# illuin-tech/colpali

Measured on AMD Instinct MI355X. Metric: MaxSim (query,doc) pairs scored/sec, higher is better.
Workload: dtype bf16; 1 GPU; 4 query x 32 tokens vs resident pre-embedded shard of 125000 docs x 1024 patches x d=128 bf16 per GPU (30.5 GiB/GPU), fused MaxSim + per-shard top-10; docs_per_gpu=125000, doc_len=1024, n_queries=4, q_len=32, top_k=10, parallelism=corpus-sharded x1

## Files before the change

colpali_amd/_lib.py:

```python
from __future__ import annotations

import ctypes
import os

import torch

_HERE = os.path.dirname(os.path.abspath(__file__))
_AB_DIR = os.path.realpath(os.path.join(_HERE, "..", "tools", "_ab"))


def _lib_path() -> str:
    override = os.environ.get("COLPALI_AMD_LIB")
    if override:
        real = os.path.realpath(override)
        if os.path.dirname(real) != _AB_DIR:
            raise RuntimeError(f"COLPALI_AMD_LIB={override}: only measurement builds under {_AB_DIR} can replace the in-tree library")
        return real
    return os.path.join(_HERE, "csrc", "libmaxsim_gfx950.so")


LIB_PATH = _lib_path()

MSIM_FLAG_REF_ROUNDING = 0x1
ABI_VERSION = 22


def dtype_code(dtype) -> int:
    if dtype == torch.bfloat16:
        return 0
    if dtype == torch.float16:
        return 1
    if dtype == torch.float32:
        return 2
    raise NotImplementedError(f"dtype {dtype}: the gfx950 kernels take bfloat16, float16 or float32 embeddings")


def kernel_width(dim: int, dtype) -> int:
    es = 4 if dtype == torch.float32 else 2
    if es == 2 and dim == 128:
        return dim
    per = 32 // es
    width = (dim + per - 1) // per * per
    if width * es > 4096:
        raise NotImplementedError(f"embedding rows of {dim} x {es} bytes exceed the 4 KiB the gfx950 kernels support")
    return width

_lib = None


class MaxSimLibraryError(RuntimeError):
    pass


def lib() -> ctypes.CDLL:
    global _lib
    if _lib is not None:
        return _lib
    if not os.path.exists(LIB_PATH):
        raise MaxSimLibraryError(
            f"{LIB_PATH} is missing: build it with `python -c 'import __graft_entry__ as g; g.build()'` "
            "(or `make -C colpali_amd/csrc`). colpali_amd has no CPU/torch fallback."
        )
    L = ctypes.CDLL(LIB_PATH)
    vp, i32, i64, u32, sz = ctypes.c_void_p, ctypes.c_int, ctypes.c_int64, ctypes.c_uint32, ctypes.c_size_t
    L.msim_abi_version.restype = i32
    L.msim_last_error.restype = ctypes.c_char_p
    L.msim_fwd_workspace_bytes.argtypes = [i32, i32, i32, i32, i32]
    L.msim_fwd_workspace_bytes.restype = sz
    L.msim_fwd.argtypes = [i32, vp, i32, i32, vp, vp, vp, i32, i32, vp, i64, u32, vp, vp]
    L.msim_fwd.restype = i32
    L.msim_fwd_host.argtypes = [i32, vp, i32, i32, vp, vp, vp, i32, i32, vp, i64, u32, i32]
    L.msim_fwd_host.restype = i32
    L.msim_host_last_error.restype = ctypes.c_char_p
    L.msim_fwd_host_lists.argtypes = [i32, vp, vp, i32, vp, vp, vp, i32, i32, vp, i64, u32, i32]
    L.msim_fwd_host_lists.restype = i32
    L.msim_sim_matrix_host.argtypes = [i32, vp, i32, vp, i32, i32, vp, i64, u32, i32]
    L.msim_sim_matrix_host.restype = i32
    L.msim_fwd_plan.argtypes = [vp, i32, i32, vp]
    L.msim_fwd_plan.restype = i32
    L.msim_fwd_ragged_workspace_bytes.argtypes = [i32, vp, i32, i32, i32]
    L.msim_fwd_ragged_workspace_bytes.restype = sz
    L.msim_fwd_ragged.argtypes = [i32, vp, vp, vp, i32, vp, vp, vp, i32, i32, vp, i64, u32, vp, vp]
    L.msim_fwd_ragged.restype = i32
    L.msim_query_compact.argtypes = [vp, i32, i32, i32, vp, vp, vp, vp]
    L.msim_query_compact.restype = i32
    L.msim_host_count_nonzero_rows.argtypes = [vp, vp, i64, i64, vp, i32]
    L.msim_host_count_nonzero_rows.restype = i32
    L.msim_host_gather_nonzero_rows.argtypes = [vp, vp, vp, i64, vp, i64, i32]
    L.msim_host_gather_nonzero_rows.restype = i32
    L.msim_fwd_transposed.argtypes = [i32, vp, i32, i32, vp, i32, i32, i32, vp, i64, vp, vp]
    L.msim_fwd_transposed.restype = i32
    L.msim_dense_t_supported.argtypes = [i32, i32, i32, i32, i32, i32]
    L.msim_dense_t_supported.restype = i32
    L.msim_dense_t_route_bytes.argtypes = [i32, i32, i32]
    L.msim_dense_t_route_bytes.restype = sz
    L.msim_fwd_transposed_route.argtypes = [i32, vp, i32, i32, vp, i32, i32, i32, vp, i64, vp, vp, vp]
    L.msim_fwd_transposed_route.restype = i32
    L.msim_dense_t_bwd_workspace_bytes.argtypes = [i32, i32, i32, i32, i32]
    L.msim_dense_t_bwd_workspace_bytes.restype = sz
    L.msim_dense_t_bwd.argtypes = [i32, vp, i32, i32, vp, i32, i32, i32, vp, i64, vp, i32, vp, vp, vp, vp, vp]
    L.msim_dense_t_bwd.restype = i32
    L.msim_host_gather_range.argtypes = [vp, vp, vp, i64, i64, i64, i32]
    L.msim_host_gather_range.restype = i32
    L.msim_host_gather_range_begin.argtypes = [vp, vp, vp, i64, i64, i64, i32]
    L.msim_host_gather_range_begin.restype = i32
    L.msim_host_gather_range_wait.argtypes = []
    L.msim_host_gather_range_wait.restype = i32
    L.msim_host_threads_affinity.argtypes = [vp, i32]
    L.msim_host_threads_affinity.restype = i32
    L.msim_pairs_argmax.argtypes = [i32, vp, i32, i32, vp, vp, vp, i32, i32, i32, vp, i32, vp, vp, vp]
    L.msim_pairs_argmax.restype = i32
    L.msim_allpairs_argmax.argtypes = [i32, vp, i32, i32, vp, vp, vp, i32, i32, vp, i64, vp, vp]
    L.msim_allpairs_argmax.restype = i32
    L.msim_pairs_bwd.argtypes = [i32, vp, i32, i32, vp, vp, i32, i32, i32, vp, vp, vp, vp, i32, vp, i32, i32, vp, vp, vp, vp]
    L.msim_pairs_bwd.restype = i32
    L.msim_pairs_bwd_workspace_bytes.argtypes = [i32, i32, i32, i32, i32, i32]
    L.msim_pairs_bwd_workspace_bytes.restype = sz
    f32 = ctypes.c_float
    L.msim_smooth_fwd.argtypes = [i32, vp, i32, i32, vp, vp, i32, i32, f32, vp, i64, vp]
    L.msim_smooth_fwd.restype = i32
    L.msim_smooth_pairs.argtypes = [i32, vp, i32, i32, vp, vp, i32, i32, vp, i32, f32, vp, vp, vp]
    L.msim_smooth_pairs.restype = i32
    L.msim_smooth_bwd_workspace_bytes.argtypes = [i32, i32, i32]
    L.msim_smooth_bwd_workspace_bytes.restype = sz
    L.msim_smooth_pairs_bwd.argtypes = [i32, vp, i32, i32, vp, vp, i32, i32, i32, vp, vp, vp, vp, i32, f32, vp, vp, vp, vp]
    L.msim_smooth_pairs_bwd.restype = i32
    L.msim_embed_head.argtypes = [i32, vp, i64, i32, vp, vp, i32, vp, vp, i64, vp]
    L.msim_embed_head.restype = i32
    L.msim_embed_head_row_map.argtypes = [vp, i32, vp, i32, i64, vp, vp]
    L.msim_embed_head_row_map.restype = i32
    L.msim_embed_head_writer_map.argtypes = [vp, i32, vp, i32, i32, i32, vp, vp, vp, vp, vp]
    L.msim_embed_head_writer_map.restype = i32
    L.msim_embed_head_bwd.argtypes = [i32, vp, vp, vp, i64, i32, vp, vp]
    L.msim_embed_head_bwd.restype = i32
    L.msim_sim_matrix.argtypes = [i32, vp, i32, vp, i32, i32, vp, i64, u32, vp]
    L.msim_sim_matrix.restype = i32
    L.msim_pool_cluster.argtypes = [i32, vp, vp, i32, i32, i32, vp, i32, vp, vp, vp, vp, vp]
    L.msim_pool_cluster.restype = i32
    L.msim_pool_reduce.argtypes = [i32, vp, vp, i32, i32, i32, vp, vp, vp, i32, vp]
    L.msim_pool_reduce.restype = i32
    L.msim_loss_epilogue_workspace_bytes.argtypes = [i32, i32]
    L.msim_loss_epilogue_workspace_bytes.restype = sz
    L.msim_loss_epilogue.argtypes = [i32, vp, i64, i32, i32, vp, i32, i32, i32, i32, f32, i32, i32, f32, f32, vp, vp, vp, vp, vp, vp, vp, vp, vp]
    L.msim_loss_epilogue.restype = i32
    L.msim_host_gather.argtypes = [vp, vp, vp, vp, i64, i32]
    L.msim_host_gather.restype = i32
    L.msim_fwd_candidates_workspace_bytes.argtypes = [i32, i32, i32]
    L.msim_fwd_candidates_workspace_bytes.restype = sz
    L.msim_fwd_candidates.argtypes = [i32, vp, vp, vp, i32, vp, vp, vp, i32, i32, vp, i32, i64, i64, vp, i64, vp, u32, vp, vp]
    L.msim_fwd_candidates.restype = i32
    L.msim_fwd_candidates_wide_workspace_bytes.argtypes = [i32, i32, i32, i32]
    L.msim_fwd_candidates_wide_workspace_bytes.restype = sz
    L.msim_fwd_candidates_wide.argtypes = L.msim_fwd_candidates.argtypes
    L.msim_fwd_candidates_wide.restype = i32
    L.msim_fde_encode_docs.argtypes = [i32, vp, vp, i32, i64, i32, vp, vp, i32, i32, i32, i32, vp, vp, vp]
    L.msim_fde_encode_docs.restype = i32
    L.msim_fde_encode_queries.argtypes = [i32, vp, vp, i32, i64, i32, vp, vp, i32, i32, i32, vp, vp, vp]
    L.msim_fde_encode_queries.restype = i32
    L.msim_fde_scores.argtypes = [i32, vp, i32, vp, i32, i32, vp, i64, vp]
    L.msim_fde_scores.restype = i32
    L.msim_i8_encode_docs.argtypes = [i32, vp, vp, i32, i64, i32, vp, vp, vp]
    L.msim_i8_encode_docs.restype = i32
    L.msim_i8_encode_queries.argtypes = [i32, vp, i64, i32, vp, vp, vp]
    L.msim_i8_encode_queries.restype = i32
    L.msim_i8_scores.argtypes = [vp, vp, vp, i32, i64, i32, vp, vp, vp, vp, i32, i64, i32, vp, i64, vp]
    L.msim_i8_scores.restype = i32
    L.msim_cent_encode_docs.argtypes = [i32, vp, vp, i32, i64, i32, i32, vp, i32, vp, vp, vp]
    L.msim_cent_encode_docs.restype = i32
    L.msim_cent_table_bytes.argtypes = [i32, i32, i32]
    L.msim_cent_table_bytes.restype = sz
    L.msim_cent_table.argtypes = [i32, vp, vp, i32, i64, i32, i32, vp, i32, vp, vp]
    L.msim_cent_table.restype = i32
    L.msim_cent_scores_plan.argtypes = [i32, i32, i32, i32, i64, vp]
    L.msim_cent_scores_plan.restype = i32
    L.msim_cent_scores.argtypes = [vp, vp, i32, i64, i32, i32, vp, vp, vp, i32, i64, vp, i64, vp]
    L.msim_cent_scores.restype = i32
    L.msim_res_encode_docs.argtypes = [i32, vp, i64, i32, vp, vp, i32, vp, i32, vp, vp]
    L.msim_res_encode_docs.restype = i32
    L.msim_res_decode_rows.argtypes = [i32, vp, vp, i64, i64, i64, vp, i32, vp, i32, i32, vp, vp]
    L.msim_res_decode_rows.restype = i32
    L.msim_res_candidates_workspace_bytes.argtypes = [i32, i32, i32]
    L.msim_res_candidates_workspace_bytes.restype = sz
    L.msim_res_candidates.argtypes = [i32, vp, vp, vp, i32, vp, vp, vp, i32, vp, i32, vp, vp, i32, i64, i32, vp, i32, i64, i64, vp, i64,
                                      vp, vp, vp]
    L.msim_res_candidates.restype = i32
    L.msim_res_scores_workspace_bytes.argtypes = [i32, i32]
    L.msim_res_scores_workspace_bytes.restype = sz
    L.msim_res_scores.argtypes = [i32, vp, vp, vp, i32, vp, vp, vp, i32, vp, i32, vp, vp, i32, i64, i32, vp, i64, vp, vp]
    L.msim_res_scores.restype = i32
    L.msim_live_compact_workspace_bytes.argtypes = [i32, i64]
    L.msim_live_compact_workspace_bytes.restype = sz
    L.msim_live_compact.argtypes = [vp, i64, i64, vp, vp, i32, vp, vp, vp, i64, vp]
    L.msim_live_compact.restype = i32
    L.msim_live_mask_scores.argtypes = [vp, i64, i32, i64, vp, vp]
    L.msim_live_mask_scores.restype = i32
    L.msim_mine_bounds.argtypes = [vp, i64, i32, i64, vp, vp, i64, i64, vp, i32, vp, vp]
    L.msim_mine_bounds.restype = i32
    L.msim_mine_mask.argtypes = [vp, i64, i32, i64, vp, f32, vp, vp, vp, i64, i64, vp]
    L.msim_mine_mask.restype = i32
    L.msim_gather_pages.argtypes = [vp, i64, i64, vp, i32, i64, vp, i64, i64, vp, vp, vp]
    L.msim_gather_pages.restype = i32
    L.msim_filter_pack.argtypes = [vp, i64, i32, i64, vp, i64, vp]
    L.msim_filter_pack.restype = i32
    L.msim_filter_mask.argtypes = [vp, i64, i32, i64, vp, i64, vp, vp, vp, vp]
    L.msim_filter_mask.restype = i32
    L.msim_filter_list_workspace_bytes.argtypes = [i32, i64]
    L.msim_filter_list_workspace_bytes.restype = sz
    L.msim_filter_list.argtypes = [vp, i64, vp, vp, vp, i32, i64, i64, vp, i64, i32, vp, vp, vp]
    L.msim_filter_list.restype = i32
    L.msim_filter_ids.argtypes = [vp, i64, i32, i64, i64, i64, vp, i64, vp, vp, vp, vp]
    L.msim_filter_ids.restype = i32
    L.msim_group_reduce.argtypes = [vp, i64, i32, i64, vp, vp, i32, i64, vp, vp, i64, vp]
    L.msim_group_reduce.restype = i32
    L.msim_group_select.argtypes = [vp, vp, vp, i32, i32, i64, i32, vp, vp, vp, vp]
    L.msim_group_select.restype = i32
    L.msim_align_candidates.argtypes =[i32, vp, vp, i32, i64, i32, vp, vp, vp, i32, i64, i32, vp, i32, i64, i64, vp, vp, vp, i32, vp]
    L.msim_align_candidates.restype = i32
    L.msim_topk_workspace_bytes.argtypes = [i32, i64, i32]
    L.msim_topk_workspace_bytes.restype = sz
    L.msim_topk_f32.argtypes = [vp, vp, i32, i64, i64, i32, i64, vp, vp, vp, vp]
    L.msim_topk_f32.restype = i32
    if L.msim_abi_version() != ABI_VERSION:
        raise MaxSimLibraryError(f"ABI version mismatch: library reports {L.msim_abi_version()}, binding expects {ABI_VERSION} "
                                 "(rebuild: make -C colpali_amd/csrc)")
    _lib = L
    return L


def check(rc: int, what: str) -> None:
    if rc != 0:
        msg = lib().msim_last_error().decode("utf-8", "replace")
        if rc == -2:
            raise NotImplementedError(f"{what}: {msg}")
        if rc == -1:
            raise ValueError(f"{what}: {msg}")
        raise MaxSimLibraryError(f"{what} failed (code {rc}): {msg}")


class StreamConstCache:

    def __init__(self, capacity: int):
        import collections
        import threading

        self._d = collections.OrderedDict()
        self._lock = threading.Lock()
        self._cap = capacity

    def get(self, key, device, make):
        k = (key, str(device), torch.cuda.current_stream(device).cuda_stream if torch.device(device).type == "cuda" else 0)
        with self._lock:
            t = self._d.get(k)
            if t is not None:
                self._d.move_to_end(k)
                return t
        t = make()
        with self._lock:
            self._d[k] = t
            while len(self._d) > self._cap:
                self._d.popitem(last=False)
        return t

    def __len__(self):
        return len(self._d)


def effective_cpus() -> int:
    try:
        n = len(os.sched_getaffinity(0))
    except Exception:
        n = os.cpu_count() or 1
    quota = None
    try:
        q, p = open("/sys/fs/cgroup/cpu.max").read().split()[:2]
        if q != "max":
            quota = int(q) / int(p)
    except Exception:
        try:
            q = int(open("/sys/fs/cgroup/cpu/cpu.cfs_quota_us").read())
            p = int(open("/sys/fs/cgroup/cpu/cpu.cfs_period_us").read())
            if q > 0 and p > 0:
                quota = q / p
        except Exception:
            pass
    if quota is not None:
        n = min(n, max(1, int(quota)))
    return max(1, n)


_gpu_cpus = {}


def _parse_cpulist(text: str):
    cpus = set()
    for part in text.strip().split(","):
        if not part:
            continue
        lo, _, hi = part.partition("-")
        cpus.update(range(int(lo), int(hi or lo) + 1))
    return cpus


def gpu_local_cpus(device):
    idx = device.index if getattr(device, "index", None) is not None else torch.cuda.current_device()
    if idx in _gpu_cpus:
        return _gpu_cpus[idx]
    cpus = None
    if os.environ.get("COLPALI_AMD_NUMA", "1") != "0":
        try:
            p = torch.cuda.get_device_properties(idx)
            bus = f"{p.pci_domain_id:04x}:{p.pci_bus_id:02x}:{p.pci_device_id:02x}.0"
            local = _parse_cpulist(open(f"/sys/bus/pci/devices/{bus}/local_cpulist").read())
            allowed = os.sched_getaffinity(0)
            local &= allowed
            if len(local) >= 2 and local != allowed:
                cpus = frozenset(local)
        except Exception:
            cpus = None
    _gpu_cpus[idx] = cpus
    return cpus


class on_gpu_local_cpus:

    def __init__(self, device):
        self.cpus = gpu_local_cpus(device) if torch.cuda.is_available() else None
        self.saved = None

    def __enter__(self):
        if self.cpus is not None:
            try:
                saved = os.sched_getaffinity(0)
                if saved != self.cpus:
                    os.sched_setaffinity(0, self.cpus)
                    self.saved = saved
            except Exception:
                self.saved = None
        return self

    def __exit__(self, *exc):
        if self.saved is not None:
            try:
                os.sched_setaffinity(0, self.saved)
            except Exception:
                pass
        return False


_SYS_MOVE_PAGES = 279


def nodes_of_addresses(addrs) -> list:
    try:
        n = len(addrs)
        if n == 0:
            return []
        libc = ctypes.CDLL(None, use_errno=True)
        pages = (ctypes.c_void_p * n)(*[int(a) & ~4095 for a in addrs])
        status = (ctypes.c_int * n)()
        libc.syscall.restype = ctypes.c_long
        rc = libc.syscall(ctypes.c_long(_SYS_MOVE_PAGES), ctypes.c_int(0), ctypes.c_ulong(n), pages, ctypes.c_void_p(0), status, ctypes.c_int(0))
        if rc != 0:
            return []
        return [int(x) for x in status if x >= 0]
    except Exception:
        return []


_node_cpus = {}


def node_cpus(node: int):
    if node in _node_cpus:
        return _node_cpus[node]
    cpus = None
    try:
        local = _parse_cpulist(open(f"/sys/devices/system/node/node{node}/cpulist").read()) & os.sched_getaffinity(0)
        if len(local) >= 2:
            cpus = frozenset(local)
    except Exception:
        cpus = None
    _node_cpus[node] = cpus
    return cpus


_gather_threads_on = [None]
GATHER_NODE_POLICY = os.environ.get("COLPALI_AMD_GATHER_NODE", "gpu")


def place_gather_threads(device, sample_addrs) -> None:
    if os.environ.get("COLPALI_AMD_NUMA", "1") == "0":
        return
    try:
        want = gpu_local_cpus(device)
        if GATHER_NODE_POLICY == "pages":
            nodes = nodes_of_addresses(sample_addrs)
            if nodes:
                node = max(set(nodes), key=nodes.count)
                want = node_cpus(node) or want
        if want is None or want == _gather_threads_on[0]:
            return
        arr = (ctypes.c_int32 * len(want))(*sorted(want))
        if lib().msim_host_threads_affinity(arr, len(want)) == 0:
            _gather_threads_on[0] = want
    except Exception:
        pass


def ptr(t) -> int:
    return 0 if t is None else t.data_ptr()


def current_stream_handle(device) -> int:
    return torch.cuda.current_stream(device).cuda_stream


def workspace(nbytes: int, device):
    return torch.empty((nbytes,), dtype=torch.uint8, device=device) if nbytes else None
```

colpali_amd/corpus.py:

```python
from __future__ import annotations

import ctypes
import operator
import os
import threading
from dataclasses import dataclass
from typing import List, Optional, Sequence, Union

import numpy as np
import torch

from . import _lib as _lib_mod
from ._lib import kernel_width

EMBED_DIM = 128


def block_clamp0(lengths: torch.Tensor, batch_size: int) -> torch.Tensor:
    if batch_size <= 0:
        raise ValueError("batch_size must be positive")
    import numpy as np

    ln = lengths.detach().to("cpu").numpy().astype(np.int64, copy=False)
    n = ln.size
    if n == 0:
        return torch.zeros((0,), dtype=torch.uint8)
    if batch_size >= n:
        flags = ln < ln.max()
    else:
        pad = (-n) % batch_size
        padded = np.concatenate([ln, np.full((pad,), -1, dtype=np.int64)]) if pad else ln
        block_max = np.repeat(padded.reshape(-1, batch_size).max(axis=1), batch_size)[:n]
        flags = ln < block_max
    return torch.from_numpy(flags.astype(np.uint8))


@dataclass
class PackedCorpus:
    blob: torch.Tensor
    offsets: torch.Tensor
    clamp0: Optional[torch.Tensor]
    lengths: torch.Tensor
    id_base: int = 0
    avg_rows: Optional[int] = None

    def __len__(self) -> int:
        return int(self.lengths.numel())

    def average_rows(self) -> int:
        if self.avg_rows is None:
            n = len(self)
            if not n:
                self.avg_rows = 0
            elif self.lengths.device.type == "cpu":
                self.avg_rows = int(self.lengths.numpy().sum(dtype=np.int64)) // n
            else:
                self.avg_rows = int(self.lengths.sum()) // n
        return self.avg_rows

    @property
    def device(self) -> torch.device:
        return self.blob.device

    @property
    def dtype(self) -> torch.dtype:
        return self.blob.dtype

    @property
    def width(self) -> int:
        return int(self.blob.shape[1])

    @property
    def nbytes(self) -> int:
        return self.blob.numel() * self.blob.element_size()


def _check_embeddings(x: torch.Tensor, what: str) -> None:
    if x.dim() not in (2, 3):
        raise ValueError(f"{what}: expected 2-D or 3-D embeddings")
    if x.dtype not in (torch.bfloat16, torch.float16, torch.float32):
        raise NotImplementedError(
            f"{what}: dtype {x.dtype}; the gfx950 kernels take bfloat16 (what the ColPali/ColQwen2 forward emits), "
            "float16 or float32 embeddings. Converting silently would change the scores, so this is an error.")
    kernel_width(x.shape[-1], x.dtype)


def _widen(x: torch.Tensor) -> torch.Tensor:
    width = kernel_width(x.shape[-1], x.dtype)
    if width == x.shape[-1]:
        return x
    return torch.nn.functional.pad(x, (0, width - x.shape[-1]))


def _env_int(name: str, default: int, lo: int, hi: int) -> int:
    try:
        return max(lo, min(hi, int(os.environ[name])))
    except (KeyError, ValueError):
        return default


_COPY_THREADS = _env_int("COLPALI_AMD_COPY_THREADS", max(1, min(8, _lib_mod.effective_cpus() // 2)), 1, 256)
_EDGE_CHUNK_BYTES = _env_int("COLPALI_AMD_EDGE_CHUNK_MB", 16, 0, 1024) << 20
_EDGE_LAST_BYTES = (lambda mb: -1 if mb < 0 else mb << 20)(_env_int("COLPALI_AMD_EDGE_LAST_MB", -1, -1, 1024))
STAGING_BYTES = _env_int("COLPALI_AMD_STAGING_MB", 64, 2, 16384) << 20
_ASYNC_GATHER = _env_int("COLPALI_AMD_ASYNC_GATHER", 1, 0, 1) == 1


class _Staging:

    def __init__(self):
        self.buf: Optional[torch.Tensor] = None
        self.events = [None, None]
        self.lock = threading.Lock()
        self.next_half = 0

    def _halves(self, want: int):
        half = max(min(want, STAGING_BYTES // 2), 1 << 20)
        if self.buf is None or self.buf.numel() < 2 * half:
            for ev in self.events:
                if ev is not None:
                    ev.synchronize()
            with _lib_mod.on_gpu_local_cpus(torch.device("cuda", torch.cuda.current_device()) if torch.cuda.is_available() else None):
                self.buf = torch.empty((2 * half,), dtype=torch.uint8, pin_memory=True)
        return self.buf.numel() // 2

    def upload(self, ps: Sequence[torch.Tensor], dim: int, device: torch.device,
               slot_rows: Optional[int] = None) -> torch.Tensor:
        dtype = ps[0].dtype
        es = ps[0].element_size()
        total = sum(int(p.shape[0]) for p in ps) if slot_rows is None else len(ps) * slot_rows
        nbytes = total * dim * es
        dev = torch.empty((total, dim), dtype=dtype, device=device)
        if nbytes == 0:
            return dev
        dev_bytes = dev.view(torch.uint8).view(-1)
        with self.lock:
            half = self._halves(nbytes)
            base = self.buf.data_ptr()
            import numpy as np

            L = _lib_mod.lib()
            keep, offs, srcs, sizes = [], [], [], []
            o = 0
            for p in ps:
                n = int(p.shape[0]) * dim * es
                if n:
                    src = p if p.is_contiguous() else p.contiguous()
                    keep.append(src)
                    sp, done = src.data_ptr(), 0
                    while done < n:
                        room = half - ((o + done) % half)
                        take = min(room, n - done)
                        offs.append(o + done)
                        srcs.append(sp + done)
                        sizes.append(take)
                        done += take
                o += n if slot_rows is None else slot_rows * dim * es
            offs_a = np.asarray(offs, dtype=np.int64)
            srcs_a = np.asarray(srcs, dtype=np.uint64)
            sizes_a = np.asarray(sizes, dtype=np.int64)
            stream = torch.cuda.current_stream(device)
            k = 0
            n_pieces = len(offs)
            for c0 in range(0, nbytes, half):
                c1 = min(nbytes, c0 + half)
                h = (c0 // half) & 1
                hb = base + h * half
                if self.events[h] is not None:
                    self.events[h].synchronize()
                if slot_rows is not None:
                    ctypes.memset(hb, 0, c1 - c0)
                k1 = k
                while k1 < n_pieces and offs[k1] < c1:
                    k1 += 1
                if k1 > k:
                    rel = offs_a[k:k1] - c0
                    rc = L.msim_host_gather(hb, srcs_a[k:k1].ctypes.data, rel.ctypes.data, sizes_a[k:k1].ctypes.data,
                                            k1 - k, _COPY_THREADS)
                    if rc != 0:
                        raise RuntimeError(f"msim_host_gather failed: {L.msim_last_error().decode()}")
                k = k1
                dev_bytes[c0:c1].copy_(self.buf[h * half : h * half + (c1 - c0)], non_blocking=True)
                self.events[h] = torch.cuda.Event()
                self.events[h].record(stream)
            del keep
        return dev


    def upload_image(self, srcs, prefix, n: int, dst_bytes: Optional[torch.Tensor], side_stream, on_chunk=None, prepare=None) -> None:
        total = int(prefix[n])
        if total == 0:
            if prepare is not None:
                prepare()
            return
        L = _lib_mod.lib()
        with self.lock:
            half = self._halves(total)
            base = self.buf.data_ptr()
            chunks = _chunk_schedule(total, half)
            in_flight = False

            def begin(k: int) -> int:
                h = self.next_half
                self.next_half ^= 1
                if self.events[h] is not None:
                    self.events[h].synchronize()
                c0, c1 = chunks[k]
                rc = L.msim_host_gather_range_begin(base + h * half, srcs.ctypes.data, prefix.ctypes.data, n, c0, c1, _COPY_THREADS)
                if rc != 0:
                    raise RuntimeError(f"msim_host_gather_range_begin failed: {L.msim_host_last_error().decode()}")
                return h

            try:
                if not _ASYNC_GATHER and prepare is not None:
                    got = prepare()
                    dst_bytes = got if dst_bytes is None else dst_bytes
                h = begin(0)
                in_flight = True
                if _ASYNC_GATHER and prepare is not None:
                    got = prepare()
                    dst_bytes = got if dst_bytes is None else dst_bytes
                for k, (c0, c1) in enumerate(chunks):
                    rc = L.msim_host_gather_range_wait()
                    in_flight = False
                    if rc != 0:
                        raise RuntimeError(f"msim_host_gather_range failed: {L.msim_host_last_error().decode()}")
                    with torch.cuda.stream(side_stream):
                        dst_bytes[c0:c1].copy_(self.buf[h * half : h * half + (c1 - c0)], non_blocking=True)
                        ev = torch.cuda.Event()
                        ev.record(side_stream)
                    self.events[h] = ev
                    if _ASYNC_GATHER and k + 1 < len(chunks):
                        h = begin(k + 1)
                        in_flight = True
                    if on_chunk is not None:
                        on_chunk(c1)
                    if not _ASYNC_GATHER and k + 1 < len(chunks):
                        h = begin(k + 1)
                        in_flight = True
            finally:
                if in_flight:
                    L.msim_host_gather_range_wait()


def _chunk_schedule(total: int, half: int):
    edge = min(_EDGE_CHUNK_BYTES, half)
    last = min(_EDGE_LAST_BYTES, half) if _EDGE_LAST_BYTES >= 0 else edge
    if edge <= 0 or last <= 0 or total <= 2 * half:
        return [(c0, min(total, c0 + half)) for c0 in range(0, total, half)]
    cuts = [0, edge]
    while total - cuts[-1] > half + last:
        cuts.append(cuts[-1] + half)
    if total - cuts[-1] > last:
        cuts.append(total - last)
    cuts.append(total)
    return list(zip(cuts[:-1], cuts[1:]))


class _PerDevice:

    def __init__(self):
        self._by_dev = {}
        self._lock = threading.Lock()

    def of(self, device) -> _Staging:
        idx = torch.device(device).index
        if idx is None:
            idx = torch.cuda.current_device() if torch.cuda.is_available() else -1
        with self._lock:
            st = self._by_dev.get(idx)
            if st is None:
                st = self._by_dev[idx] = _Staging()
            return st

    def upload(self, ps, dim, device, slot_rows=None):
        return self.of(device).upload(ps, dim, device, slot_rows)


_staging = _PerDevice()
_staging_q = _PerDevice()
_copy_streams = {}


def copy_stream(device: torch.device) -> torch.cuda.Stream:
    device = torch.device(device)
    key = device.index if device.index is not None else torch.cuda.current_device()
    st = _copy_streams.get(key)
    if st is None:
        st = _copy_streams[key] = torch.cuda.Stream(device=device)
    return st


_dim_of = torch.Tensor.dim
_dtype_of = operator.attrgetter("dtype")
_shape_of = operator.attrgetter("shape")
_is_cpu = operator.attrgetter("is_cpu")
_is_contig = torch.Tensor.is_contiguous
_data_ptr = torch.Tensor.data_ptr
_stride_of = torch.Tensor.stride
_numel_of = torch.Tensor.numel


def host_list_image(ps: Sequence[torch.Tensor], what: str = "passages"):
    first = ps[0]
    dtype, dim = first.dtype, (first.shape[1] if first.dim() == 2 else -1)
    if dim > 0 and type(ps) in (list, tuple):
        n = len(ps)
        if (set(map(_dim_of, ps)) == {2} and set(map(_dtype_of, ps)) == {dtype} and all(map(_is_cpu, ps))
                and all(map(_is_contig, ps)) and set(map(_stride_of, ps)) == {(dim, 1)}):
            numel = np.fromiter(map(_numel_of, ps), dtype=np.int64, count=n)
            rows = numel // dim
            if bool((rows >= 2).all()) and bool((rows * dim == numel).all()):
                _check_embeddings(first, what)
                srcs = np.fromiter(map(_data_ptr, ps), dtype=np.uint64, count=n)
                return list(ps), srcs, rows, int(dim), dtype
    keep = []
    for p in ps:
        if p.dim() != 2:
            raise ValueError(f"each {what[:-1]} must be 2-D (sequence_length, dim)")
        if p.dtype != dtype:
            raise RuntimeError(f"expected {what} of one dtype, got {dtype} and {p.dtype}")
        if p.shape[1] != dim:
            raise RuntimeError(f"expected {what} of one embedding width, got {dim} and {p.shape[1]}")
        if p.device.type != "cpu":
            return None
        keep.append(p if p.is_contiguous() else p.contiguous())
    _check_embeddings(first, what)
    srcs = np.fromiter((t.data_ptr() for t in keep), dtype=np.uint64, count=len(keep))
    rows = np.fromiter((t.shape[0] for t in keep), dtype=np.int64, count=len(keep))
    return keep, srcs, rows, int(dim), dtype


def _gather_rows(ps: Sequence[torch.Tensor], dim: int, device: torch.device) -> torch.Tensor:
    device = torch.device(device)
    if device.type == "cuda" and all(p.device.type == "cpu" for p in ps):
        return _staging.upload(ps, dim, device)
    return torch.cat([p.reshape(-1, dim) for p in ps], dim=0).to(device, non_blocking=True)


def pack_passages(ps: Union[torch.Tensor, Sequence[torch.Tensor]], device: torch.device,
                  batch_size: Optional[int] = 128, id_base: int = 0) -> PackedCorpus:
    if isinstance(ps, torch.Tensor):
        if ps.dim() != 3:
            raise ValueError("a passage tensor must be 3-D (n_passages, max_len, dim)")
        _check_embeddings(ps, "passages")
        n, L, dim = ps.shape
        blob = _widen(ps.reshape(n * L, dim).to(device, non_blocking=True)).contiguous()
        lengths = torch.full((n,), L, dtype=torch.int64)
        clamp0 = None
    else:
        if len(ps) == 0:
            raise ValueError("No passages provided")
        for p in ps:
            if p.dim() != 2:
                raise ValueError("each passage must be 2-D (sequence_length, dim)")
            _check_embeddings(p, "passages")
            if p.dtype != ps[0].dtype:
                raise RuntimeError(f"expected passages of one dtype, got {ps[0].dtype} and {p.dtype}")
            if p.shape[1] != ps[0].shape[1]:
                raise RuntimeError(f"expected passages of one embedding width, got {ps[0].shape[1]} and {p.shape[1]}")
        dim = ps[0].shape[1]
        lengths = torch.tensor([p.shape[0] for p in ps], dtype=torch.int64)
        blob = _widen(_gather_rows(ps, dim, device)).contiguous()
        clamp0 = None
        if batch_size is not None:
            flags = block_clamp0(lengths, batch_size)
            if bool(flags.any()):
                clamp0 = flags.to(device)
            if bool((lengths == 0).any()):
                for j in range(0, len(ps), batch_size):
                    if int(lengths[j : j + batch_size].max()) == 0:
                        raise RuntimeError("max(): Expected reduction dim 3 to have non-zero size.")
    if blob.numel() == 0:
        blob = torch.zeros((1, blob.shape[1]), dtype=blob.dtype, device=device)
    offsets = torch.zeros(lengths.numel() + 1, dtype=torch.int64)
    torch.cumsum(lengths, 0, out=offsets[1:])
    if int(offsets[-1]) >= 2**31:
        raise NotImplementedError("more than 2^31 patch rows in one shard")
    return PackedCorpus(blob=blob, offsets=offsets.to(torch.int32).to(device), clamp0=clamp0,
                        lengths=lengths, id_base=id_base)


@dataclass
class PackedQueries:
    tokens: torch.Tensor
    offsets: torch.Tensor
    offsets_host: torch.Tensor

    def __len__(self) -> int:
        return int(self.offsets_host.numel()) - 1

    @property
    def device(self) -> torch.device:
        return self.tokens.device

    @property
    def dtype(self) -> torch.dtype:
        return self.tokens.dtype

    @property
    def lengths(self) -> torch.Tensor:
        return (self.offsets_host[1:] - self.offsets_host[:-1]).to(torch.int64)

    def select(self, lo: int, hi: int) -> "PackedQueries":
        base = int(self.offsets_host[lo])
        oh = (self.offsets_host[lo:hi + 1] - base).contiguous()
        return PackedQueries(tokens=self.tokens[base:int(self.offsets_host[hi])] if hi > lo else self.tokens[:0],
                             offsets=oh.to(self.tokens.device, non_blocking=True), offsets_host=oh)


MAX_FLAT_QUERY_TOKENS = 1024
WIDE_DIM = 320
MAX_FLAT_QUERY_TOKENS_WIDE = 512


def _is_flat_shape(dtype: torch.dtype, dim: int) -> bool:
    return dtype in (torch.bfloat16, torch.float16) and dim in (EMBED_DIM, WIDE_DIM)


def max_flat_query_tokens(dim: int) -> int:
    return MAX_FLAT_QUERY_TOKENS_WIDE if dim == WIDE_DIM else MAX_FLAT_QUERY_TOKENS


def _flat_from_host_list(qs: Sequence[torch.Tensor], dim: int, device: torch.device, compact: bool) -> Optional["PackedQueries"]:
    import numpy as np

    L = _lib_mod.lib()
    es = qs[0].element_size()
    row_bytes = dim * es
    keep = [q if q.is_contiguous() else q.contiguous() for q in qs]
    n = len(keep)
    srcs = np.asarray([q.data_ptr() for q in keep], dtype=np.uint64)
    rows = np.asarray([int(q.shape[0]) for q in keep], dtype=np.int64)
    if compact:
        counts = np.zeros(n, dtype=np.int32)
        rc = L.msim_host_count_nonzero_rows(srcs.ctypes.data, rows.ctypes.data, row_bytes, n, counts.ctypes.data, _COPY_THREADS)
        if rc != 0:
            raise RuntimeError(f"msim_host_count_nonzero_rows failed: {L.msim_last_error().decode()}")
    else:
        counts = rows.astype(np.int32)
    if int(counts.max(initial=0)) > max_flat_query_tokens(dim):
        return None
    off = np.zeros(n + 1, dtype=np.int64)
    np.cumsum(counts, out=off[1:])
    total = int(off[-1])
    offsets_host = torch.from_numpy(off.astype(np.int32))
    tokens = torch.empty((max(total, 1), dim), dtype=qs[0].dtype, device=device)
    if total == 0:
        tokens.zero_()
    else:
        st = _staging_q.of(device)
        stream = torch.cuda.current_stream(device)
        dst_bytes = tokens.view(torch.uint8).view(-1)
        if not compact:
            prefix = np.zeros(n + 1, dtype=np.int64)
            np.cumsum(rows * row_bytes, out=prefix[1:])
            st.upload_image(srcs, prefix, n, dst_bytes[:total * row_bytes], stream)
        else:
            with st.lock:
                half = st._halves(total * row_bytes)
                base = st.buf.data_ptr()
                g0 = 0
                while g0 < n:
                    g1 = g0 + 1
                    while g1 < n and (off[g1 + 1] - off[g0]) * row_bytes <= half:
                        g1 += 1
                    nb = int(off[g1] - off[g0]) * row_bytes
                    if nb:
                        h = st.next_half
                        st.next_half ^= 1
                        if st.events[h] is not None:
                            st.events[h].synchronize()
                        dst_row = np.ascontiguousarray(off[g0:g1] - off[g0])
                        rc = L.msim_host_gather_nonzero_rows(base + h * half, srcs[g0:g1].ctypes.data, rows[g0:g1].ctypes.data, row_bytes,
                                                             dst_row.ctypes.data, g1 - g0, _COPY_THREADS)
                        if rc != 0:
                            raise RuntimeError(f"host query gather failed: {L.msim_last_error().decode()}")
                        lo = int(off[g0]) * row_bytes
                        dst_bytes[lo:lo + nb].copy_(st.buf[h * half: h * half + nb], non_blocking=True)
                        ev = torch.cuda.Event()
                        ev.record(stream)
                        st.events[h] = ev
                    g0 = g1
    del keep
    return PackedQueries(tokens=tokens, offsets=offsets_host.to(device, non_blocking=True), offsets_host=offsets_host)


def _flat_from_device_box(box: torch.Tensor, compact: bool) -> Optional["PackedQueries"]:
    n_q, Lq, dim = box.shape
    box = box.contiguous()
    if not compact or n_q == 0 or Lq == 0:
        if Lq > max_flat_query_tokens(dim):
            return None
        oh = (torch.arange(n_q + 1, dtype=torch.int64) * Lq).to(torch.int32)
        tok = box.reshape(n_q * Lq, dim)
        if tok.shape[0] == 0:
            tok = torch.zeros((1, dim), dtype=box.dtype, device=box.device)
        return PackedQueries(tokens=tok, offsets=oh.to(box.device, non_blocking=True), offsets_host=oh)
    if Lq > 4096:
        return None
    L = _lib_mod.lib()
    row_bytes = dim * box.element_size()
    counts = torch.empty((n_q,), dtype=torch.int32, device=box.device)
    with torch.cuda.device(box.device):
        stream = _lib_mod.current_stream_handle(box.device)
        _lib_mod.check(L.msim_query_compact(_lib_mod.ptr(box), n_q, Lq, row_bytes, None, _lib_mod.ptr(counts), None, stream),
                       "msim_query_compact")
        counts_h = counts.cpu()
        if int(counts_h.max()) > max_flat_query_tokens(dim):
            return None
        oh = torch.zeros(n_q + 1, dtype=torch.int32)
        torch.cumsum(counts_h, 0, out=oh[1:])
        off = oh.to(box.device, non_blocking=True)
        total = int(oh[-1])
        tokens = torch.empty((max(total, 1), dim), dtype=box.dtype, device=box.device)
        if total == 0:
            tokens.zero_()
        else:
            _lib_mod.check(L.msim_query_compact(_lib_mod.ptr(box), n_q, Lq, row_bytes, _lib_mod.ptr(off), None, _lib_mod.ptr(tokens),
                                                stream), "msim_query_compact")
    return PackedQueries(tokens=tokens, offsets=off, offsets_host=oh)


def check_query_list(qs: Sequence[torch.Tensor]) -> None:
    if len(qs) == 0:
        raise ValueError("No queries provided")
    for q in qs:
        if q.dim() != 2:
            raise ValueError("each query must be 2-D (sequence_length, dim)")
        _check_embeddings(q, "queries")
        if q.dtype != qs[0].dtype:
            raise RuntimeError(f"expected queries of one dtype, got {qs[0].dtype} and {q.dtype}")
        if q.shape[1] != qs[0].shape[1]:
            raise RuntimeError(f"expected queries of one embedding width, got {qs[0].shape[1]} and {q.shape[1]}")


def pack_queries(qs: Union[torch.Tensor, Sequence[torch.Tensor]], device: torch.device, *, layout: str = "auto",
                 compact: bool = True, _checked: bool = False) -> Union[torch.Tensor, "PackedQueries"]:
    if layout not in ("auto", "flat", "box"):
        raise ValueError("layout must be 'auto', 'flat' or 'box'")
    device = torch.device(device)
    if isinstance(qs, torch.Tensor):
        if qs.dim() != 3:
            raise ValueError("a query tensor must be 3-D (n_queries, max_len, dim)")
        _check_embeddings(qs, "queries")
        if layout != "box" and device.type == "cuda" and _is_flat_shape(qs.dtype, qs.shape[2]):
            flat = _flat_from_device_box(qs.to(device, non_blocking=True), compact)
            if flat is not None:
                return flat
        if layout == "flat":
            raise NotImplementedError("the flat query layout takes bf16 / f16 embeddings of width 128 (320) on the GPU, at most "
                                      f"{MAX_FLAT_QUERY_TOKENS} ({MAX_FLAT_QUERY_TOKENS_WIDE}) tokens per query")
        return _widen(qs.to(device, non_blocking=True)).contiguous()
    if not _checked:
        check_query_list(qs)
    dim = int(qs[0].shape[1])
    if layout != "box" and device.type == "cuda" and _is_flat_shape(qs[0].dtype, dim):
        if all(q.device.type == "cpu" for q in qs):
            flat = _flat_from_host_list(qs, dim, device, compact)
        else:
            l_max = max(int(q.shape[0]) for q in qs)
            box = torch.nn.utils.rnn.pad_sequence([q.to(device) for q in qs], batch_first=True, padding_value=0) if l_max else None
            flat = _flat_from_device_box(box, True) if box is not None else None
        if flat is not None:
            return flat
    if layout == "flat":
        raise NotImplementedError("the flat query layout takes bf16 / f16 embeddings of width 128 (320) on the GPU, at most "
                                  f"{MAX_FLAT_QUERY_TOKENS} ({MAX_FLAT_QUERY_TOKENS_WIDE}) tokens per query")
    if device.type == "cuda" and all(q.device.type == "cpu" for q in qs):
        l_max = max(int(q.shape[0]) for q in qs)
        if l_max == 0:
            padded = torch.zeros((len(qs), 0, dim), dtype=qs[0].dtype, device=device)
        else:
            padded = _staging_q.upload(qs, dim, device, slot_rows=l_max).view(len(qs), l_max, dim)
    else:
        padded = torch.nn.utils.rnn.pad_sequence(list(qs), batch_first=True, padding_value=0).to(device, non_blocking=True)
    return _widen(padded).contiguous()


def _dtype_width(queries):
    if isinstance(queries, PackedQueries):
        return queries.dtype, int(queries.tokens.shape[1])
    if isinstance(queries, torch.Tensor):
        return queries.dtype, int(queries.shape[-1])
    if len(queries) == 0:
        raise ValueError("No queries provided")
    return queries[0].dtype, int(queries[0].shape[-1])


def _as_packed(queries, device: torch.device, *, layout: str = "auto", compact: bool = False):
    if isinstance(queries, PackedQueries):
        return queries
    dense_on_device = isinstance(queries, torch.Tensor) and queries.device.type == "cuda"
    return pack_queries(queries, device, layout=layout, compact=compact or not dense_on_device)


def _id_list(ids, n_q: int, device: torch.device, what: str):
    if not isinstance(ids, torch.Tensor) or ids.dtype != torch.int64 or ids.dim() != 2 or ids.shape[0] != n_q or ids.device != device:
        raise ValueError(f"{what} must be an int64 [n_q={n_q}, m] tensor on {device}")
    m = int(ids.shape[1])
    if (m > 1 and ids.stride(1) != 1) or (n_q > 1 and ids.stride(0) < m):
        ids = ids.contiguous()
    return ids, m, ids.stride(0) if n_q > 1 else max(m, 1)


def _rerank_args(n_q: int, device: torch.device, candidates, out, ws_bytes):
    candidates, m, ld = _id_list(candidates, n_q, device, "candidates")
    if out is None:
        out = torch.empty((n_q, m), dtype=torch.float32, device=device)
    elif out.shape != (n_q, m) or out.dtype != torch.float32 or not out.is_contiguous() or out.device != device:
        raise ValueError("out must be a contiguous fp32 [n_q, m] tensor on the corpus' device")
    ids = torch.empty((n_q, m), dtype=torch.int64, device=device)
    return candidates, m, ld, out, ids, _lib_mod.workspace(int(ws_bytes(m)), device)
```

colpali_amd/csrc/maxsim_abi.hip:

```cpp
#include <hip/hip_runtime.h>

#include <atomic>
#include <cstdlib>
#include <cstring>
#include <type_traits>
#include <vector>

#include "../../include/maxsim.h"
#include "abi_common.hpp"
#include "abi_shapes.hpp"
#include "maxsim_stream.hip"
#include "maxsim_batch.hip"
#if defined(MSIM_AB) || defined(MSIM_TRACE)
#include "maxsim_batch_packed.hip"
#endif
#include "maxsim_generic.hip"
#include "maxsim_panels.hip"
#include "maxsim_candidates.hip"
#include "maxsim_candidates_panels.hip"
#include "query_compact.hip"

using namespace msim_abi;

namespace {

struct FwdCall {
    const uint16_t *Q, *D;
    const int32_t *d_off;
    const uint8_t *clamp0;
    float *scores;
    long long ld;
    int n_q, Lq, n_d;
    unsigned flags;
    const DeviceInfo *di;
    hipStream_t st;
    void *workspace = nullptr;
    const int32_t *q_off = nullptr;
    const int32_t *q_off_host = nullptr;
    int seg = 0, n_seg = 1;
    int avg_rows = 0;
};

constexpr size_t kFwdWorkspaceBytes = 4096;

constexpr int kStreamRing = 4;

struct HostQ {
    const int32_t *off;
    int Lq, seg, n_seg;
    int at(int i) const {
        if (off) return off[i];
        if (n_seg <= 1) return i * Lq;
        const int r = i / n_seg, s = i - r * n_seg;
        const int o = s * seg;
        return r * Lq + (o < Lq ? o : Lq);
    }
};
HostQ host_q(const FwdCall &c) { return HostQ{c.q_off_host, c.Lq, c.seg, c.n_seg}; }
msim::FlatQ flat_q(const FwdCall &c) { return msim::FlatQ{c.q_off, c.Lq, c.seg, c.n_seg}; }

int stream_nt() {
    static const int v = ab_env("MSIM_STREAM_NT", 1) != 0;
    return v;
}

template <int NU, bool F16, int AUX, bool IL, int RING = kStreamRing>
int launch_stream_aux(const FwdCall &c) {
    auto kern = msim::maxsim_stream_kernel<NU, RING, F16, AUX, IL>;
    constexpr int lds = 4 * (RING * msim::kSlabBytes + msim::kStreamTokBytes);
    static std::atomic<int> configured[kMaxDevices];
    if (int rc = allow_lds(kern, lds, configured)) return rc;
    msim::StreamArgs a;
    a.ld = c.ld;
    a.fq = flat_q(c);
    a.n_q = c.n_q;
    a.n_d = c.n_d;
    a.flags = c.flags;
    const int wg_needed = (c.n_d + 3) / 4;
    const int wg_cap = c.di->cus * (c.di->lds_per_cu / lds);
    hipLaunchKernelGGL(kern, dim3(wg_needed < wg_cap ? wg_needed : wg_cap), dim3(256), lds, c.st, c.Q, c.D, c.d_off,
                       c.clamp0, c.scores, a);
    hipError_t e = hipGetLastError();
    if (e != hipSuccess) return fail(MSIM_ELAUNCH, "maxsim_stream_kernel<%d> launch: %s", NU, hipGetErrorString(e));
    return MSIM_OK;
}

int stream_il() {
    static const int v = ab_env("MSIM_STREAM_IL", 1) != 0;
    return v;
}

template <int NU, bool F16>
int launch_stream(const FwdCall &c) {
    constexpr int ring_default = NU >= 5 ? 2 : kStreamRing;
#ifdef MSIM_AB
    {
        static const int ring_env = ab_env("MSIM_STREAM_RING", 0);
        const int ring = ring_env ? ring_env : ring_default;
        if (ring == 2) return launch_stream_aux<NU, F16, 2, true, 2>(c);
        if (stream_il() && stream_nt()) return launch_stream_aux<NU, F16, 2, true>(c);
        return stream_nt() ? launch_stream_aux<NU, F16, 2, false>(c) : launch_stream_aux<NU, F16, 0, false>(c);
    }
#endif
    return launch_stream_aux<NU, F16, 2, true, ring_default>(c);
}

struct FlatPlan {
    bool stream = false;
    int nu = 0;
    int nw = 0, maxu = 0;
    std::vector<int> blk_q0;
    int n_blocks() const { return (int)blk_q0.size() - 1; }
};

bool fill_blocks(const HostQ &hq, int n_q, int nw, int maxu, std::vector<int> &blk) {
    const int cap_tok = nw * maxu * msim::kUnitTok, cap_q = nw * 8;
    blk.clear();
    blk.push_back(0);
    int cur_tok = 0, cur_q = 0;
    for (int i = 0; i < n_q; ++i) {
        const int len = hq.at(i + 1) - hq.at(i);
        if (len > cap_tok) return false;
        if (cur_q == cap_q || cur_tok + len > cap_tok) {
            blk.push_back(i);
            cur_tok = 0;
            cur_q = 0;
        }
        cur_tok += len;
        ++cur_q;
    }
    blk.push_back(n_q);
    return true;
}

void balance_blocks(const HostQ &hq, int n_q, int nw, int maxu, std::vector<int> &blk) {
    const int nb = (int)blk.size() - 1;
    if (nb <= 1) return;
    const int cap_tok = nw * maxu * msim::kUnitTok, cap_q = nw * 8;
    const long long base = hq.at(0), total = (long long)hq.at(n_q) - base;
    std::vector<int> cut(1, 0);
    int q = 0;
    for (int b = 1; b < nb; ++b) {
        const long long want = (total * b + nb - 1) / nb;
        while (q < n_q && (long long)hq.at(q) - base < want) ++q;
        if (q <= cut.back()) q = cut.back() + 1;
        if (q >= n_q) return;
        cut.push_back(q);
    }
    cut.push_back(n_q);
    for (int b = 0; b < nb; ++b)
        if (hq.at(cut[b + 1]) - hq.at(cut[b]) > cap_tok || cut[b + 1] - cut[b] > cap_q) return;
    blk.swap(cut);
}

int heaviest_wave_units(const HostQ &hq, const std::vector<int> &blk, int nw) {
    int worst = 0;
    for (size_t b = 0; b + 1 < blk.size(); ++b) {
        const int units = (hq.at(blk[b + 1]) - hq.at(blk[b]) + msim::kUnitTok - 1) / msim::kUnitTok;
        const int w = (units + nw - 1) / nw;
        if (w > worst) worst = w;
    }
    return worst;
}

int batch_nw_override() {
    static const int v = [] {
        const int x = ab_env("MSIM_BATCH_NW", 0);
        return (x == 2 || x == 4 || x == 8) ? x : 0;
    }();
    return v;
}

int flat_plan(const HostQ &hq, int n_q, FlatPlan &p) {
    const long long tokens = (long long)hq.at(n_q) - hq.at(0);
    if (tokens < 0) return fail(MSIM_EINVAL, "query token offsets are not non-decreasing");
    const long long units = (tokens + msim::kUnitTok - 1) / msim::kUnitTok;
    p = FlatPlan{};
    if (n_q <= 8 && units <= 8) {
        p.stream = true;
        p.nu = units > 0 ? (int)units : 1;
        return MSIM_OK;
    }
    static const int shapes[7][2] = {{2, 8}, {4, 5}, {2, 10}, {4, 8}, {4, 10}, {8, 8}, {8, 10}};
    const int forced = batch_nw_override();
    static const int forced_maxu = ab_env("MSIM_BATCH_MAXU", 0);
#ifdef MSIM_AB
    if (forced == 2 && forced_maxu == 5 && units <= 10 && n_q <= 16 && fill_blocks(hq, n_q, 2, 5, p.blk_q0) && p.n_blocks() == 1) {
        p.nw = 2;
        p.maxu = 5;
        return MSIM_OK;
    }
#endif
    for (const auto &sh : shapes) {
        if (forced && sh[0] != forced) continue;
        if (forced_maxu && sh[1] != forced_maxu) continue;
        if (units > sh[0] * sh[1] || n_q > sh[0] * 8) continue;
        if (sh[0] == 2 && sh[1] == 10 && !(forced == 2 || forced_maxu == 10)) continue;
        if (!fill_blocks(hq, n_q, sh[0], sh[1], p.blk_q0) || p.n_blocks() != 1) continue;
        p.nw = sh[0];
        p.maxu = sh[1];
        return MSIM_OK;
    }
#ifdef MSIM_AB
    if (forced == 4) {
        std::vector<int> b4;
        if (fill_blocks(hq, n_q, 4, 8, b4)) {
            balance_blocks(hq, n_q, 4, 8, b4);
            p.nw = 4;
            p.maxu = 8;
            p.blk_q0.swap(b4);
            return MSIM_OK;
        }
    }
#endif
    std::vector<int> b8, b10;
    if (!fill_blocks(hq, n_q, 8, 8, b8)) {
        if (!fill_blocks(hq, n_q, 8, 10, b10))
            return fail(MSIM_EUNSUPPORTED, "a query of more than %d tokens does not fit one query block", 8 * 10 * msim::kUnitTok);
        balance_blocks(hq, n_q, 8, 10, b10);
        p.nw = 8;
        p.maxu = 10;
        p.blk_q0.swap(b10);
        return MSIM_OK;
    }
    balance_blocks(hq, n_q, 8, 8, b8);
    p.nw = 8;
    p.maxu = 8;
    if (fill_blocks(hq, n_q, 8, 10, b10)) {
        balance_blocks(hq, n_q, 8, 10, b10);
        const long long c8 = (long long)(b8.size() - 1) * heaviest_wave_units(hq, b8, 8);
        const long long c10 = (long long)(b10.size() - 1) * heaviest_wave_units(hq, b10, 8);
        const bool single_round10 = b10.size() - 1 <= 32 && b10.size() - 1 >= 31 && b8.size() - 1 > 32;
        if (11 * c10 < 10 * c8 || (c10 <= c8 && single_round10)) {
            p.maxu = 10;
            p.blk_q0.swap(b10);
            return MSIM_OK;
        }
    }
    p.blk_q0.swap(b8);
    return MSIM_OK;
}

int ranges_per_xcd(int n_qblocks, int cus_per_xcd, int n_d, int avg_rows) {
    int min_docs = 64;
    if (avg_rows > 0) {
        min_docs = (2048 + avg_rows - 1) / avg_rows;
        min_docs = min_docs < 2 ? 2 : (min_docs > 64 ? 64 : min_docs);
    }
    int sub = n_qblocks >= cus_per_xcd ? 1 : cus_per_xcd / n_qblocks;
    if (n_qblocks > 1) {
        double best = 0.0;
        int best_sub = 1;
        for (int s = 1; s <= 32; ++s) {
            if (s > 1 && (long long)8 * s * min_docs > n_d) break;
            const long long slots_x = (long long)n_qblocks * s;
            const long long rounds = (slots_x + cus_per_xcd - 1) / cus_per_xcd;
            const double eff = (double)slots_x / (double)(rounds * cus_per_xcd);
            if (eff > best + 1e-9) {
                best = eff;
                best_sub = s;
            }
            if (eff >= (s == 1 ? 0.93 : 0.97)) break;
        }
        sub = best_sub;
    }
    return sub;
}

template <bool F16, int NW, int RING, int AUX, int MAXU, bool PACKED>
auto batch_kernel_ptr() {
#if defined(MSIM_AB) || defined(MSIM_TRACE)
    if constexpr (PACKED) return msim::maxsim_batch_packed_kernel<F16, AUX, MAXU>;
    else
#endif
    return msim::maxsim_batch_kernel<F16, NW, RING, AUX, MAXU>;
}

template <bool F16, int NW, int RING = 3, int AUX = 0, int MAXU = 8, bool PACKED = false>
int launch_batch(const FwdCall &c, const FlatPlan &plan) {
    static_assert(!PACKED || (NW == 8 && RING == 3), "K1bK is the eight-wave form");
    auto kern = batch_kernel_ptr<F16, NW, RING, AUX, MAXU, PACKED>();
    constexpr int lds = RING * (NW / 2) * msim::kSlabBytes +
                        (PACKED ? 2 * (NW / 2) * NW * MAXU * msim::kUnitTok * 4 : (NW > 2 ? 2 : 1) * NW * MAXU * msim::kUnitTok * 16) +
                        NW * 8 * 8;
    constexpr int wg_per_cu = MAXU == 5 ? 12 / NW : 8 / NW;
    static std::atomic<int> configured[kMaxDevices];
    if (int rc = allow_lds(kern, lds, configured)) return rc;
    const int cus_per_xcd = (c.di->cus / 8 > 0 ? c.di->cus / 8 : 1) * wg_per_cu;
    static const int over_env = ab_env("MSIM_BATCH_OVER", NW == 4 ? 8 : 1);
    static const bool convoy_off = ab_env("MSIM_BATCH_CONVOY", 1) == 0;
    const int total_blocks = plan.n_blocks();
    for (int b0 = 0; b0 < total_blocks; b0 += msim::kMaxQBlocks) {
        msim::BatchArgs a{};
        a.ld = c.ld;
        a.fq = flat_q(c);
        a.n_d = c.n_d;
        a.flags = c.flags;
        a.n_qblocks = total_blocks - b0 < msim::kMaxQBlocks ? total_blocks - b0 : msim::kMaxQBlocks;
        for (int b = 0; b <= a.n_qblocks; ++b) a.blk_q0[b] = plan.blk_q0[b0 + b];
        int sub = ranges_per_xcd(a.n_qblocks, cus_per_xcd, c.n_d, c.avg_rows);
        if (NW < 8 && a.n_qblocks == 1 && over_env > 1) {
            int over = over_env;
            while (over > 1 && (long long)8 * sub * over * 16 > c.n_d) over >>= 1;
            sub *= over;
        }
        a.n_ranges = 8 * sub;
        const int slots = sub > 1 ? a.n_qblocks * sub : a.n_qblocks;
        a.convoy = nullptr;
        if (c.workspace && !convoy_off && a.n_qblocks > 1 && (long long)a.n_qblocks * sub <= cus_per_xcd && a.n_qblocks <= 64 &&
            (size_t)a.n_ranges * a.n_qblocks * sizeof(int) <= kFwdWorkspaceBytes) {
            a.convoy = static_cast<int *>(c.workspace);
            if (hipMemsetAsync(a.convoy, 0, (size_t)a.n_ranges * a.n_qblocks * sizeof(int), c.st) != hipSuccess)
                return fail(MSIM_ELAUNCH, "hipMemsetAsync(convoy counters) failed");
        }
        a.trace = nullptr;
#ifdef MSIM_TRACE
        if (const char *tp = getenv("MSIM_BATCH_TRACE_PTR")) a.trace = reinterpret_cast<unsigned long long *>(strtoull(tp, nullptr, 0));
#endif
        hipLaunchKernelGGL(kern, dim3(8 * slots), dim3(NW * 64), lds, c.st, c.Q, c.D, c.d_off, c.clamp0, c.scores, a);
        hipError_t e = hipGetLastError();
        if (e != hipSuccess) return fail(MSIM_ELAUNCH, "maxsim_batch%s_kernel<%d,%d> launch: %s", PACKED ? "_packed" : "", NW, MAXU, hipGetErrorString(e));
    }
    return MSIM_OK;
}

template <bool F16>
int fwd_dispatch(const FwdCall &c) {
    thread_local FlatPlan plan;
    if (int rc = flat_plan(host_q(c), c.n_q, plan)) return rc;
    if (plan.stream) {
        switch (plan.nu) {
            case 1: return launch_stream<1, F16>(c);
            case 2: return launch_stream<2, F16>(c);
            case 3: return launch_stream<3, F16>(c);
            case 4: return launch_stream<4, F16>(c);
            case 5: return launch_stream<5, F16>(c);
            case 6: return launch_stream<6, F16>(c);
            case 7: return launch_stream<7, F16>(c);
            default: return launch_stream<8, F16>(c);
        }
    }
    static const bool nt_off = ab_env("MSIM_BATCH_NT", 1) == 0;
    const bool single = plan.n_blocks() == 1 && !nt_off;
    if (plan.nw == 4 && plan.maxu == 5) {
#ifdef MSIM_AB
        static const int ring5 = ab_env("MSIM_BATCH_RING5", 2);
        if (ring5 == 3) return launch_batch<F16, 4, 3, 2, 5>(c, plan);
#endif
        return launch_batch<F16, 4, 2, 2, 5>(c, plan);
    }
#ifdef MSIM_AB
    if (plan.nw == 2 && plan.maxu == 10) return launch_batch<F16, 2, 4, 2, 10>(c, plan);
    if (plan.nw == 2 && plan.maxu == 5) {
        static const int ring5p = ab_env("MSIM_BATCH_RING5", 2);
        return ring5p == 3 ? launch_batch<F16, 2, 3, 2, 5>(c, plan) : launch_batch<F16, 2, 2, 2, 5>(c, plan);
    }
#endif
    if (plan.nw == 2) return launch_batch<F16, 2, 4, 2, 8>(c, plan);
#ifdef MSIM_AB
    if (plan.nw == 4 && plan.maxu == 8 && !single) return launch_batch<F16, 4, 3, 0, 8>(c, plan);
#endif
    if (plan.nw == 4) return plan.maxu == 10 ? launch_batch<F16, 4, 3, 2, 10>(c, plan) : launch_batch<F16, 4, 3, 2, 8>(c, plan);
#if defined(MSIM_AB) || defined(MSIM_TRACE)
    static const int packed_env = ab_env("MSIM_BATCH_PACKED", 0);
    if (packed_env != 0) {
        if (plan.maxu == 10) return single ? launch_batch<F16, 8, 3, 2, 10, true>(c, plan) : launch_batch<F16, 8, 3, 0, 10, true>(c, plan);
        return single ? launch_batch<F16, 8, 3, 2, 8, true>(c, plan) : launch_batch<F16, 8, 3, 0, 8, true>(c, plan);
    }
#endif
    if (plan.maxu == 10) return single ? launch_batch<F16, 8, 3, 2, 10>(c, plan) : launch_batch<F16, 8, 3, 0, 10>(c, plan);
    return single ? launch_batch<F16, 8, 3, 2, 8>(c, plan) : launch_batch<F16, 8, 3, 0, 8>(c, plan);
}

size_t flat_workspace_bytes(const HostQ &hq, int n_q) {
    thread_local FlatPlan plan;
    if (flat_plan(hq, n_q, plan) != MSIM_OK) return 0;
    return (!plan.stream && plan.n_blocks() > 1) ? kFwdWorkspaceBytes : 0;
}

template <int DT, int T>
int launch_generic(const GenericCall &c) {
    auto kern = msim::maxsim_generic_kernel<DT, T>;
    const int lds = T * msim::kTokTile * (c.row_bytes + 16);
    static std::atomic<int> configured[kMaxDevices];
    if (int rc = allow_lds(kern, 160 * 1024, configured)) return rc;
    msim::GenericArgs a;
    a.ld = c.ld;
    a.n_q = c.n_q;
    a.Lq = c.Lq;
    a.n_d = c.n_d;
    a.row_bytes = c.row_bytes;
    a.flags = c.flags;
    const int tpq = (c.Lq + msim::kTokTile - 1) / msim::kTokTile;
    const int groups = tpq <= T ? (c.n_q + (T / tpq) - 1) / (T / tpq) : c.n_q;
    if (groups > 65535) return fail(MSIM_EUNSUPPORTED, "too many query groups (%d) for one launch", groups);
    const int wg_needed = (c.n_d + msim::kGenericWaves - 1) / msim::kGenericWaves;
    int per_cu = c.di->lds_per_cu / lds;
    per_cu = per_cu < 1 ? 1 : (per_cu > 4 ? 4 : per_cu);
    const int wg_cap = c.di->cus * per_cu;
    hipLaunchKernelGGL(kern, dim3(wg_needed < wg_cap ? wg_needed : wg_cap, groups), dim3(msim::kGenericWaves * 64), lds, c.st,
                       c.Q, c.D, c.d_off, c.clamp0, c.scores, a);
    hipError_t e = hipGetLastError();
    if (e != hipSuccess) return fail(MSIM_ELAUNCH, "maxsim_generic_kernel<%d,%d> launch: %s", DT, T, hipGetErrorString(e));
    return MSIM_OK;
}

template <int DT>
int generic_dispatch(const GenericCall &c) {
    const int tpq = (c.Lq + msim::kTokTile - 1) / msim::kTokTile;
    const long long tiles = (long long)c.n_q * tpq;
    const int tile_lds = msim::kTokTile * (c.row_bytes + 16);
    int T = 4;
    while (T > 1 && (T * tile_lds > 96 * 1024 || T / 2 >= tiles)) T >>= 1;
    switch (T) {
        case 4: return launch_generic<DT, 4>(c);
        case 2: return launch_generic<DT, 2>(c);
        default: return launch_generic<DT, 1>(c);
    }
}

int generic_fwd(int dtype, const GenericCall &c) {
    switch (dtype) {
        case MSIM_DTYPE_F32: return generic_dispatch<msim::kDtypeF32>(c);
        case MSIM_DTYPE_F16: return generic_dispatch<msim::kDtypeF16>(c);
        default: return generic_dispatch<msim::kDtypeBf16>(c);
    }
}


template <int DT, int T>
int launch_sim(const char *A, const char *B, float *out, const msim::SimArgs &a, const DeviceInfo &di, hipStream_t st) {
    auto kern = msim::sim_matrix_kernel<DT, T>;
    const int lds = T * msim::kTokTile * (a.row_bytes + 16);
    static std::atomic<int> configured[kMaxDevices];
    if (int rc = allow_lds(kern, 160 * 1024, configured)) return rc;
    const int groups = (a.n_a + T * msim::kTokTile - 1) / (T * msim::kTokTile);
    if (groups > 65535) return fail(MSIM_EUNSUPPORTED, "too many row groups (%d) for one launch", groups);
    const int slabs = (a.n_b + msim::kSlabRows - 1) / msim::kSlabRows;
    const int wg_needed = (slabs + msim::kGenericWaves - 1) / msim::kGenericWaves;
    int per_cu = di.lds_per_cu / lds;
    per_cu = per_cu < 1 ? 1 : (per_cu > 4 ? 4 : per_cu);
    const int wg_cap = di.cus * per_cu;
    hipLaunchKernelGGL(kern, dim3(wg_needed < wg_cap ? wg_needed : wg_cap, groups), dim3(msim::kGenericWaves * 64), lds, st, A, B,
                       out, a);
    hipError_t e = hipGetLastError();
    if (e != hipSuccess) return fail(MSIM_ELAUNCH, "sim_matrix_kernel<%d,%d> launch: %s", DT, T, hipGetErrorString(e));
    return MSIM_OK;
}

template <int DT>
int sim_dispatch(const char *A, const char *B, float *out, const msim::SimArgs &a, const DeviceInfo &di, hipStream_t st) {
    const int tile_lds = msim::kTokTile * (a.row_bytes + 16);
    int T = 4;
    while (T > 1 && (T * tile_lds > 80 * 1024 || (T / 2) * msim::kTokTile >= a.n_a)) T >>= 1;
    switch (T) {
        case 4: return launch_sim<DT, 4>(A, B, out, a, di, st);
        case 2: return launch_sim<DT, 2>(A, B, out, a, di, st);
        default: return launch_sim<DT, 1>(A, B, out, a, di, st);
    }
}

constexpr int kPanels320 = 3, kLast320 = 4;

bool is_panels(int dtype, int dim, long long tiles, int tpq) {
    if (!(dtype == MSIM_DTYPE_BF16 || dtype == MSIM_DTYPE_F16) || dim != 320 || tpq > 4) return false;
    return tiles <= 4 || tpq <= 2;
}

template <int QT, int TPQ, bool F16>
int launch_stream_panels(const FwdCall &c) {
    auto kern = msim::maxsim_stream_panels_kernel<QT, TPQ, kPanels320, kLast320, F16, 2>;
    constexpr int lds = 4 * msim::kPanelRing * msim::kSlabBytes;
    static std::atomic<int> configured[kMaxDevices];
    if (int rc = allow_lds(kern, lds, configured)) return rc;
    msim::PanelStreamArgs a;
    a.ld = c.ld;
    a.n_q = c.n_q;
    a.Lq = c.Lq;
    a.n_d = c.n_d;
    a.flags = c.flags;
    const int wg_needed = (c.n_d + 3) / 4;
    const int wg_cap = c.di->cus * (c.di->lds_per_cu / lds);
    hipLaunchKernelGGL(kern, dim3(wg_needed < wg_cap ? wg_needed : wg_cap), dim3(256), lds, c.st, c.Q, c.D, c.d_off, c.clamp0,
                       c.scores, a);
    hipError_t e = hipGetLastError();
    if (e != hipSuccess) return fail(MSIM_ELAUNCH, "maxsim_stream_panels_kernel<%d,%d> launch: %s", QT, TPQ, hipGetErrorString(e));
    return MSIM_OK;
}

template <int NT, int TPQ, bool F16>
int launch_batch_panels(const FwdCall &c) {
    auto kern = msim::maxsim_batch_panels_kernel<NT, TPQ, kPanels320, kLast320, F16>;
    constexpr int lds = msim::kPanelStages * kPanels320 * msim::kSlabBytes;
    static std::atomic<int> configured[kMaxDevices];
    if (int rc = allow_lds(kern, lds, configured)) return rc;
    msim::PanelBatchArgs a{};
    a.ld = c.ld;
    a.n_q = c.n_q;
    a.Lq = c.Lq;
    a.n_d = c.n_d;
    a.flags = c.flags;
    const int q_per_block = msim::kBatchWaves * NT / TPQ;
    a.n_qblocks = (c.n_q + q_per_block - 1) / q_per_block;
    const int cus_per_xcd = c.di->cus / 8 > 0 ? c.di->cus / 8 : 1;
    const int sub = a.n_qblocks >= cus_per_xcd ? 1 : cus_per_xcd / a.n_qblocks;
    a.n_ranges = 8 * sub;
    const int slots = sub > 1 ? a.n_qblocks * sub : a.n_qblocks;
    hipLaunchKernelGGL(kern, dim3(8 * slots), dim3(512), lds, c.st, c.Q, c.D, c.d_off, c.clamp0, c.scores, a);
    hipError_t e = hipGetLastError();
    if (e != hipSuccess) return fail(MSIM_ELAUNCH, "maxsim_batch_panels_kernel<%d,%d> launch: %s", NT, TPQ, hipGetErrorString(e));
    return MSIM_OK;
}

template <bool F16>
int panels_dispatch(const FwdCall &c) {
    const int tpq = (c.Lq + msim::kTokTile - 1) / msim::kTokTile;
    if ((long long)c.n_q * tpq <= 4) {
        switch (c.n_q * 10 + tpq) {
            case 11: return launch_stream_panels<1, 1, F16>(c);
            case 21: return launch_stream_panels<2, 1, F16>(c);
            case 31: return launch_stream_panels<3, 1, F16>(c);
            case 41: return launch_stream_panels<4, 1, F16>(c);
            case 12: return launch_stream_panels<2, 2, F16>(c);
            case 22: return launch_stream_panels<4, 2, F16>(c);
            case 13: return launch_stream_panels<3, 3, F16>(c);
            default: return launch_stream_panels<4, 4, F16>(c);
        }
    }
    if (tpq == 2) return launch_batch_panels<2, 2, F16>(c);
    return c.n_q <= 8 ? launch_batch_panels<1, 1, F16>(c) : launch_batch_panels<2, 1, F16>(c);
}


constexpr int kPanelsFlatMaxU = 4;
constexpr int kPanelsFlatMaxTokens = msim::kBatchWaves * kPanelsFlatMaxU * msim::kUnitTok;

int panels_flat_plan(const HostQ &hq, int n_q, FlatPlan &p) {
    if ((long long)hq.at(n_q) - hq.at(0) < 0) return fail(MSIM_EINVAL, "query token offsets are not non-decreasing");
    p = FlatPlan{};
    const long long tokens = (long long)hq.at(n_q) - hq.at(0);
    const long long units = (tokens + msim::kUnitTok - 1) / msim::kUnitTok;
    p.nw = (units <= 2 * kPanelsFlatMaxU && n_q <= 16) ? 2 : (units <= 4 * kPanelsFlatMaxU && n_q <= 32) ? 4 : msim::kBatchWaves;
    p.maxu = kPanelsFlatMaxU;
    if (!fill_blocks(hq, n_q, p.nw, p.maxu, p.blk_q0) || (p.nw != msim::kBatchWaves && p.n_blocks() != 1)) {
        p.nw = msim::kBatchWaves;
        p.blk_q0.clear();
    }
    if (p.blk_q0.empty() && !fill_blocks(hq, n_q, p.nw, p.maxu, p.blk_q0))
        return fail(MSIM_EUNSUPPORTED, "a query of more than %d tokens does not fit one query block of the width-320 kernels: pad the "
                    "queries to one length and call msim_fwd", kPanelsFlatMaxTokens);
    balance_blocks(hq, n_q, p.nw, p.maxu, p.blk_q0);
    return MSIM_OK;
}

template <bool F16, int NW, int STAGES>
int launch_batch_panels_flat_nw(const FwdCall &c, const FlatPlan &plan) {
    auto kern = msim::maxsim_batch_panels_flat_kernel<F16, kPanels320, kLast320, kPanelsFlatMaxU, NW, STAGES>;
    constexpr int lds = STAGES * kPanels320 * msim::kSlabBytes + NW * kPanelsFlatMaxU * msim::kUnitTok * 16 +
                        NW * 8 * 8;
    static std::atomic<int> configured[kMaxDevices];
    if (int rc = allow_lds(kern, lds, configured)) return rc;
    const int cus_per_xcd = (c.di->cus / 8 > 0 ? c.di->cus / 8 : 1) * (NW == msim::kBatchWaves ? 1 : 2);
    const int total_blocks = plan.n_blocks();
    for (int b0 = 0; b0 < total_blocks; b0 += msim::kMaxQBlocks) {
        msim::BatchArgs a{};
        a.ld = c.ld;
        a.fq = flat_q(c);
        a.n_d = c.n_d;
        a.flags = c.flags;
        a.n_qblocks = total_blocks - b0 < msim::kMaxQBlocks ? total_blocks - b0 : msim::kMaxQBlocks;
        for (int b = 0; b <= a.n_qblocks; ++b) a.blk_q0[b] = plan.blk_q0[b0 + b];
        const int sub = ranges_per_xcd(a.n_qblocks, cus_per_xcd, c.n_d, c.avg_rows);
        a.n_ranges = 8 * sub;
        const int slots = sub > 1 ? a.n_qblocks * sub : a.n_qblocks;
        a.convoy = nullptr;
        a.trace = nullptr;
        hipLaunchKernelGGL(kern, dim3(8 * slots), dim3(NW * 64), lds, c.st, c.Q, c.D, c.d_off, c.clamp0, c.scores, a);
        hipError_t e = hipGetLastError();
        if (e != hipSuccess) return fail(MSIM_ELAUNCH, "maxsim_batch_panels_flat_kernel<%d> launch: %s", NW, hipGetErrorString(e));
    }
    return MSIM_OK;
}

template <bool F16>
int launch_batch_panels_flat(const FwdCall &c) {
    thread_local FlatPlan plan;
    if (int rc = panels_flat_plan(host_q(c), c.n_q, plan)) return rc;
    if (plan.nw == 2) return launch_batch_panels_flat_nw<F16, 2, 3>(c, plan);
    if (plan.nw == 4) return launch_batch_panels_flat_nw<F16, 4, 3>(c, plan);
    return launch_batch_panels_flat_nw<F16, msim::kBatchWaves, msim::kPanelStages>(c, plan);
}

bool box_on_panels_flat(int dtype, int dim, int n_q, int Lq) {
    if (!(dtype == MSIM_DTYPE_BF16 || dtype == MSIM_DTYPE_F16) || dim != 320 || Lq > kPanelsFlatMaxTokens) return false;
    const int tpq = (Lq + msim::kTokTile - 1) / msim::kTokTile;
    if ((long long)n_q * tpq <= 4) return false;
    static const int forced = ab_env("MSIM_PANELS_FLAT", -1);
    if (forced == 0) return tpq > 2;
    if (forced == 1) return true;
    return tpq > 2 || (Lq % msim::kTokTile) != 0;
}

}

extern "C" {

size_t msim_fwd_workspace_bytes(int dtype, int n_q, int Lq, int n_d, int dim) {
    if (n_q <= 0 || n_d <= 0 || Lq <= 0) return 0;
    if (is_long_tuned(dtype, dim, Lq))
        return kFwdWorkspaceBytes + (size_t)n_q * long_segments(Lq) * n_d * sizeof(float);
    if (!is_tuned(dtype, dim, Lq)) return 0;
    return flat_workspace_bytes(HostQ{nullptr, Lq, 0, 1}, n_q);
}

int msim_fwd_plan(const int32_t *q_off_host, int n_q, int Lq, int32_t *out5) {
    if (!out5 || n_q <= 0 || (!q_off_host && Lq <= 0)) return fail(MSIM_EINVAL, "bad arguments");
    thread_local FlatPlan plan;
    const HostQ hq = q_off_host ? HostQ{q_off_host, 0, 0, 1}
                                : (Lq > kLongSegRows ? HostQ{nullptr, Lq, kLongSegRows, long_segments(Lq)} : HostQ{nullptr, Lq, 0, 1});
    if (!q_off_host && Lq > kLongSegRows && (long long)n_q * long_segments(Lq) > 0x7fffffff / 8)
        return fail(MSIM_EUNSUPPORTED, "too many 128-token pieces (%d queries x %d)", n_q, long_segments(Lq));
    const int n = (!q_off_host && Lq > kLongSegRows) ? n_q * long_segments(Lq) : n_q;
    if (int rc = flat_plan(hq, n, plan)) return rc;
    out5[0] = plan.stream ? 0 : 1;
    out5[1] = plan.stream ? plan.nu : plan.nw;
    out5[2] = plan.stream ? 0 : plan.maxu;
    out5[3] = plan.stream ? 1 : plan.n_blocks();
    out5[4] = plan.stream ? plan.nu : heaviest_wave_units(hq, plan.blk_q0, plan.nw);
    return MSIM_OK;
}

size_t msim_fwd_ragged_workspace_bytes(int dtype, const int32_t *q_off_host, int n_q, int n_d, int dim) {
    if (n_q <= 0 || n_d <= 0 || !q_off_host) return 0;
    if (!(dtype == MSIM_DTYPE_BF16 || dtype == MSIM_DTYPE_F16) || dim != msim::kDim) return 0;
    return flat_workspace_bytes(HostQ{q_off_host, 0, 0, 1}, n_q);
}

int msim_fwd_ragged(int dtype, const void *Qt, const int32_t *q_off, const int32_t *q_off_host, int n_q, const void *D,
                    const int32_t *d_off, const uint8_t *d_clamp0, int n_d, int dim, float *scores, int64_t ld_scores,
                    uint32_t flags, void *workspace, void *stream) {
    if (n_q < 0 || n_d < 0) return fail(MSIM_EINVAL, "negative size (n_q=%d n_d=%d)", n_q, n_d);
    if (n_q == 0 || n_d == 0) return MSIM_OK;
    if (!scores || !Qt || !D || !d_off || !q_off || !q_off_host) return fail(MSIM_EINVAL, "null pointer argument");
    if (!(dtype == MSIM_DTYPE_BF16 || dtype == MSIM_DTYPE_F16) || !(dim == msim::kDim || dim == 320))
        return fail(MSIM_EUNSUPPORTED, "msim_fwd_ragged takes bfloat16 / float16 embeddings of width %d or 320 (dtype code %d, dim %d): "
                    "pad the queries to one length and call msim_fwd", msim::kDim, dtype, dim);
    if ((reinterpret_cast<uintptr_t>(Qt) | reinterpret_cast<uintptr_t>(D)) & 15) return fail(MSIM_EINVAL, "Qt and D must be 16-byte aligned");
    if (workspace && (reinterpret_cast<uintptr_t>(workspace) & 15)) return fail(MSIM_EINVAL, "workspace must be 16-byte aligned");
    if (ld_scores < n_d) return fail(MSIM_EINVAL, "ld_scores=%lld < n_d=%d", (long long)ld_scores, n_d);
    const int avg_rows = (int)((flags >> 8) & 0xffffu);
    flags &= ~(0xffffu << 8);
    if (flags & ~(MSIM_FLAG_REF_ROUNDING)) return fail(MSIM_EINVAL, "unknown flags 0x%x", flags);
    if (q_off_host[0] != 0) return fail(MSIM_EINVAL, "q_off[0] must be 0");
    for (int i = 0; i < n_q; ++i)
        if (q_off_host[i + 1] < q_off_host[i]) return fail(MSIM_EINVAL, "q_off must be non-decreasing (query %d)", i);
    FwdCall c;
    if (int rc = device_info(&c.di)) return rc;
    c.Q = static_cast<const uint16_t *>(Qt);
    c.D = static_cast<const uint16_t *>(D);
    c.d_off = d_off;
    c.clamp0 = d_clamp0;
    c.scores = scores;
    c.ld = ld_scores;
    c.n_q = n_q;
    c.Lq = 0;
    c.n_d = n_d;
    c.flags = flags;
    c.st = static_cast<hipStream_t>(stream);
    c.workspace = workspace;
    c.q_off = q_off;
    c.q_off_host = q_off_host;
    c.avg_rows = avg_rows;
    if (dim == 320) {
        const int L0 = q_off_host[1];
        bool uniform = true;
        for (int i = 1; i < n_q && uniform; ++i) uniform = q_off_host[i + 1] - q_off_host[i] == L0;
        const int tpq = (L0 + msim::kTokTile - 1) / msim::kTokTile;
        if (uniform && L0 > 0 && is_panels(dtype, dim, (long long)n_q * tpq, tpq) && (long long)n_q * tpq <= 4) {
            c.Lq = L0;
            c.q_off = nullptr;
            c.q_off_host = nullptr;
            return dtype == MSIM_DTYPE_F16 ? panels_dispatch<true>(c) : panels_dispatch<false>(c);
        }
        return dtype == MSIM_DTYPE_F16 ? launch_batch_panels_flat<true>(c) : launch_batch_panels_flat<false>(c);
    }
    return dtype == MSIM_DTYPE_F16 ? fwd_dispatch<true>(c) : fwd_dispatch<false>(c);
}

int msim_fwd(int dtype, const void *Q, int n_q, int Lq, const void *D, const int32_t *d_off, const uint8_t *d_clamp0,
             int n_d, int dim, float *scores, int64_t ld_scores, uint32_t flags, void *workspace, void *stream) {
    if (n_q < 0 || n_d < 0 || Lq <= 0) return fail(MSIM_EINVAL, "negative size (n_q=%d n_d=%d Lq=%d)", n_q, n_d, Lq);
    if (n_q == 0 || n_d == 0) return MSIM_OK;
    if (!scores) return fail(MSIM_EINVAL, "null pointer argument");
    if (int rc = check_common(Q, D, d_off, dtype, dim, Lq)) return rc;
    if (ld_scores < n_d) return fail(MSIM_EINVAL, "ld_scores=%lld < n_d=%d", (long long)ld_scores, n_d);
    const int avg_rows = (int)((flags >> 8) & 0xffffu);
    flags &= ~(0xffffu << 8);
    if (flags & ~(MSIM_FLAG_REF_ROUNDING)) return fail(MSIM_EINVAL, "unknown flags 0x%x", flags);
    {
        const int tpq = (Lq + msim::kTokTile - 1) / msim::kTokTile;
        const bool on_flat = box_on_panels_flat(dtype, dim, n_q, Lq);
        if (on_flat || is_panels(dtype, dim, (long long)n_q * tpq, tpq)) {
            FwdCall c;
            if (int rc = device_info(&c.di)) return rc;
            c.Q = static_cast<const uint16_t *>(Q);
            c.D = static_cast<const uint16_t *>(D);
            c.d_off = d_off;
            c.clamp0 = d_clamp0;
            c.scores = scores;
            c.ld = ld_scores;
            c.n_q = n_q;
            c.Lq = Lq;
            c.n_d = n_d;
            c.flags = flags;
            c.avg_rows = avg_rows;
            c.st = static_cast<hipStream_t>(stream);
            if (on_flat)
                return dtype == MSIM_DTYPE_F16 ? launch_batch_panels_flat<true>(c) : launch_batch_panels_flat<false>(c);
            return dtype == MSIM_DTYPE_F16 ? panels_dispatch<true>(c) : panels_dispatch<false>(c);
        }
    }
    if (is_long_tuned(dtype, dim, Lq) && workspace != nullptr && (long long)n_q * long_segments(Lq) <= 0x7fffffff / 8) {
        if (reinterpret_cast<uintptr_t>(workspace) & 15) return fail(MSIM_EINVAL, "workspace must be 16-byte aligned");
        const int n_seg = long_segments(Lq);
        float *partial = reinterpret_cast<float *>(static_cast<char *>(workspace) + kFwdWorkspaceBytes);
        FwdCall c;
        if (int rc = device_info(&c.di)) return rc;
        c.Q = static_cast<const uint16_t *>(Q);
        c.D = static_cast<const uint16_t *>(D);
        c.d_off = d_off;
        c.clamp0 = d_clamp0;
        c.scores = partial;
        c.ld = n_d;
        c.n_q = n_q * n_seg;
        c.Lq = Lq;
        c.n_d = n_d;
        c.flags = flags | msim::kFlagPartial;
        c.avg_rows = avg_rows;
        c.st = static_cast<hipStream_t>(stream);
        c.workspace = workspace;
        c.seg = kLongSegRows;
        c.n_seg = n_seg;
        const bool f16 = dtype == MSIM_DTYPE_F16;
        if (int rc = f16 ? fwd_dispatch<true>(c) : fwd_dispatch<false>(c)) return rc;
        const bool round_total = (flags & MSIM_FLAG_REF_ROUNDING) != 0;
        for (int q0 = 0; q0 < n_q; q0 += 65535) {
            const int nq = n_q - q0 < 65535 ? n_q - q0 : 65535;
            const dim3 grid((n_d + 255) / 256, nq);
            const float *part = partial + (size_t)q0 * n_seg * n_d;
            float *out = scores + (size_t)q0 * ld_scores;
            if (f16)
                hipLaunchKernelGGL(msim::segment_sum_kernel<true>, grid, dim3(256), 0, c.st, part, (long long)n_d, n_seg, n_d, out,
                                   (long long)ld_scores, round_total);
            else
                hipLaunchKernelGGL(msim::segment_sum_kernel<false>, grid, dim3(256), 0, c.st, part, (long long)n_d, n_seg, n_d, out,
                                   (long long)ld_scores, round_total);
        }
        hipError_t e = hipGetLastError();
        if (e != hipSuccess) return fail(MSIM_ELAUNCH, "segment_sum_kernel launch: %s", hipGetErrorString(e));
        return MSIM_OK;
    }
    if (!is_tuned(dtype, dim, Lq)) {
        GenericCall c;
        if (int rc = device_info(&c.di)) return rc;
        c.Q = static_cast<const char *>(Q);
        c.D = static_cast<const char *>(D);
        c.d_off = d_off;
        c.clamp0 = d_clamp0;
        c.scores = scores;
        c.ld = ld_scores;
        c.n_q = n_q;
        c.Lq = Lq;
        c.n_d = n_d;
        c.row_bytes = dim * elem_bytes(dtype);
        c.flags = flags;
        c.st = static_cast<hipStream_t>(stream);
        return generic_fwd(dtype, c);
    }
    FwdCall c;
    if (int rc = device_info(&c.di)) return rc;
    c.Q = static_cast<const uint16_t *>(Q);
    c.D = static_cast<const uint16_t *>(D);
    c.d_off = d_off;
    c.clamp0 = d_clamp0;
    c.scores = scores;
    c.ld = ld_scores;
    c.n_q = n_q;
    c.Lq = Lq;
    c.n_d = n_d;
    c.flags = flags;
    c.avg_rows = avg_rows;
    c.st = static_cast<hipStream_t>(stream);
    c.workspace = workspace;
    return dtype == MSIM_DTYPE_F16 ? fwd_dispatch<true>(c) : fwd_dispatch<false>(c);
}

int msim_sim_matrix(int dtype, const void *A, int n_a, const void *B, int n_b, int dim, float *out, int64_t ld_out,
                    uint32_t flags, void *stream) {
    if (n_a < 0 || n_b < 0) return fail(MSIM_EINVAL, "negative size (n_a=%d n_b=%d)", n_a, n_b);
    if (n_a == 0 || n_b == 0) return MSIM_OK;
    if (!out) return fail(MSIM_EINVAL, "null pointer argument");
    static const int32_t dummy_off[2] = {0, 0};
    if (int rc = check_smooth(A, B, dummy_off, dtype, dim, 1, 1.0f)) return rc;
    if (ld_out < n_b) return fail(MSIM_EINVAL, "ld_out=%lld < n_b=%d", (long long)ld_out, n_b);
    if (flags & ~(MSIM_FLAG_REF_ROUNDING)) return fail(MSIM_EINVAL, "unknown flags 0x%x", flags);
    const DeviceInfo *di = nullptr;
    if (int rc = device_info(&di)) return rc;
    msim::SimArgs a{ld_out, n_a, n_b, dim * elem_bytes(dtype), flags};
    const char *ac = static_cast<const char *>(A), *bc = static_cast<const char *>(B);
    hipStream_t st = static_cast<hipStream_t>(stream);
    switch (dtype) {
        case MSIM_DTYPE_F32: return sim_dispatch<msim::kDtypeF32>(ac, bc, out, a, *di, st);
        case MSIM_DTYPE_F16: return sim_dispatch<msim::kDtypeF16>(ac, bc, out, a, *di, st);
        default: return sim_dispatch<msim::kDtypeBf16>(ac, bc, out, a, *di, st);
    }
}

int msim_query_compact(const void *box, int n_q, int Lq, int row_bytes, const int32_t *q_off, int32_t *counts, void *out,
                       void *stream) {
    if (n_q < 0 || Lq < 0 || row_bytes <= 0 || (row_bytes & 15)) return fail(MSIM_EINVAL, "bad size (row bytes must be a multiple of 16)");
    if (n_q == 0 || Lq == 0) return MSIM_OK;
    if (!box || (!counts && !(q_off && out))) return fail(MSIM_EINVAL, "null pointer argument");
    if (Lq > msim::kCompactMaxRows) return fail(MSIM_EUNSUPPORTED, "query boxes of more than %d rows are not compacted", msim::kCompactMaxRows);
    if (reinterpret_cast<uintptr_t>(box) & 15 || reinterpret_cast<uintptr_t>(out) & 15) return fail(MSIM_EINVAL, "buffers must be 16-byte aligned");
    hipLaunchKernelGGL(msim::query_compact_kernel, dim3(n_q), dim3(256), 0, static_cast<hipStream_t>(stream),
                       static_cast<const char *>(box), Lq, row_bytes, q_off, counts, static_cast<char *>(out));
    return launch_failed("query_compact_kernel");
}

}

namespace {

struct CandLayout {
    size_t status, cnt, bsum, estart, istart, rank, entries, items, total;
};

CandLayout cand_layout(int n_q, int m, int n_d) {
    const size_t E = (size_t)n_q * (size_t)m;
    const size_t nb = ((size_t)n_d + msim::kCandScanDocs - 1) / msim::kCandScanDocs;
    CandLayout L;
    size_t w = 0;
    L.status = w;   w += 16;
    L.cnt = w;      w += align16((size_t)n_d * msim::kCandClasses * 4);
    L.bsum = w;     w += align16((2 * nb + 2) * 4);
    L.estart = w;   w += align16(((size_t)n_d + 1) * 4);
    L.istart = w;   w += align16(((size_t)n_d + 1) * 4);
    L.rank = w;     w += align16(E * 4);
    L.entries = w;  w += align16(E * sizeof(int2));
    L.items = w;    w += align16(E * sizeof(msim::CandItem));
    L.total = w;
    return L;
}

int fwd_candidates(const char *who, int width, int dtype, const void *Qt, const int32_t *q_off, const int32_t *q_off_host, int n_q,
                   const void *D, const int32_t *d_off, const uint8_t *d_clamp0, int n_d, int dim, const int64_t *cand, int m,
                   int64_t ld_cand, int64_t id_base, float *out_scores, int64_t ld_scores, int64_t *out_ids, unsigned flags,
                   void *workspace, void *stream) {
    if (n_q < 0 || m < 0 || n_d < 0) return fail(MSIM_EINVAL, "negative size (n_q=%d m=%d n_d=%d)", n_q, m, n_d);
    if (n_q == 0 || m == 0) return MSIM_OK;
    if (!Qt || !q_off || !q_off_host || (!D && n_d > 0) || !d_off || !cand || !out_scores || !workspace)
        return fail(MSIM_EINVAL, "null pointer argument");
    if (!(dtype == MSIM_DTYPE_BF16 || dtype == MSIM_DTYPE_F16) || dim != width)
        return fail(MSIM_EUNSUPPORTED, "%s takes bfloat16 / float16 embeddings of width %d (dtype code %d, dim %d)", who, width, dtype,
                    dim);
    if ((reinterpret_cast<uintptr_t>(Qt) | reinterpret_cast<uintptr_t>(D) | reinterpret_cast<uintptr_t>(workspace)) & 15)
        return fail(MSIM_EINVAL, "Qt, D and workspace must be 16-byte aligned");
    if (ld_cand < m) return fail(MSIM_EINVAL, "ld_cand=%lld < m=%d", (long long)ld_cand, m);
    if (ld_scores < m) return fail(MSIM_EINVAL, "ld_scores=%lld < m=%d", (long long)ld_scores, m);
    if (flags & ~(MSIM_FLAG_REF_ROUNDING)) return fail(MSIM_EINVAL, "unknown flags 0x%x", flags);
    if ((long long)n_q * m > 0x7fffffff) return fail(MSIM_EUNSUPPORTED, "more than 2^31 - 1 entries (n_q=%d x m=%d)", n_q, m);
    if (q_off_host[0] != 0) return fail(MSIM_EINVAL, "q_off[0] must be 0");
    for (int i = 0; i < n_q; ++i) {
        const int len = q_off_host[i + 1] - q_off_host[i];
        if (len < 0) return fail(MSIM_EINVAL, "q_off must be non-decreasing (query %d)", i);
        if (len > msim::kStreamMaxUnits * msim::kUnitTok)
            return fail(MSIM_EUNSUPPORTED, "query %d has %d tokens: %s takes queries of at most %d", i, len, who,
                        msim::kStreamMaxUnits * msim::kUnitTok);
    }
    const DeviceInfo *di = nullptr;
    if (int rc = device_info(&di)) return rc;
    hipStream_t st = static_cast<hipStream_t>(stream);
    const CandLayout lay = cand_layout(n_q, m, n_d);
    char *ws = static_cast<char *>(workspace);
    int32_t *status = reinterpret_cast<int32_t *>(ws + lay.status);
    int32_t *cnt = reinterpret_cast<int32_t *>(ws + lay.cnt), *bsum = reinterpret_cast<int32_t *>(ws + lay.bsum);
    int32_t *estart = reinterpret_cast<int32_t *>(ws + lay.estart), *istart = reinterpret_cast<int32_t *>(ws + lay.istart);
    int32_t *rank = reinterpret_cast<int32_t *>(ws + lay.rank);
    int2 *entries = reinterpret_cast<int2 *>(ws + lay.entries);
    msim::CandItem *items = reinterpret_cast<msim::CandItem *>(ws + lay.items);
    const long long E = (long long)n_q * m;
    const unsigned eblocks = (unsigned)((E + 255) / 256);
    {
        const long long n16 = (long long)(lay.bsum - lay.status) / 16;
        const long long blocks = (n16 + 255) / 256;
        hipLaunchKernelGGL(msim::cand_zero_kernel, dim3((unsigned)(blocks < 1024 ? blocks : 1024)), dim3(256), 0, st,
                           reinterpret_cast<msim::i32x4 *>(status), n16);
    }
    hipLaunchKernelGGL(msim::cand_count_kernel, dim3(eblocks), dim3(256), 0, st, cand, (long long)ld_cand, n_q, m, (long long)id_base, n_d,
                       q_off, cnt, rank, out_scores, (long long)ld_scores, out_ids, status);
    hipError_t e = hipGetLastError();
    if (e != hipSuccess) return fail(MSIM_ELAUNCH, "cand_count_kernel launch: %s", hipGetErrorString(e));
    if (n_d == 0) return MSIM_OK;
    const int nb = (n_d + msim::kCandScanDocs - 1) / msim::kCandScanDocs;
    hipLaunchKernelGGL(msim::cand_block_sums_kernel, dim3(nb), dim3(256), 0, st, cnt, n_d, bsum);
    hipLaunchKernelGGL(msim::cand_scan_sums_kernel, dim3(1), dim3(256), 0, st, bsum, nb);
    hipLaunchKernelGGL(msim::cand_block_starts_kernel, dim3(nb), dim3(256), 0, st, cnt, n_d, bsum, nb, estart, istart);
    hipLaunchKernelGGL(msim::cand_place_kernel, dim3(eblocks), dim3(256), 0, st, cand, (long long)ld_cand, n_q, m, (long long)id_base, q_off,
                       cnt, rank, estart, istart, n_d, entries, items, status);
    e = hipGetLastError();
    if (e != hipSuccess) return fail(MSIM_ELAUNCH, "candidate list kernels launch: %s", hipGetErrorString(e));
    const bool f16 = dtype == MSIM_DTYPE_F16;
    const bool wide = width != msim::kDim;
    auto kern = wide ? (f16 ? msim::maxsim_candidates_panels_kernel<3, 4, true, 0> : msim::maxsim_candidates_panels_kernel<3, 4, false, 0>)
                     : (f16 ? msim::maxsim_candidates_kernel<true, 0> : msim::maxsim_candidates_kernel<false, 0>);
    const int lds_bytes = wide ? msim::kCandPanelLdsBytes : msim::kCandLdsBytes;
    static std::atomic<int> configured[2][2][kMaxDevices];
    if (int rc = allow_lds(kern, lds_bytes, configured[wide][f16])) return rc;
    const long long wg_needed = (E + 3) / 4;
    const long long wg_cap = (long long)di->cus * (di->lds_per_cu / lds_bytes);
    hipLaunchKernelGGL(kern, dim3((unsigned)(wg_needed < wg_cap ? wg_needed : wg_cap)), dim3(256), lds_bytes, st,
                       static_cast<const uint16_t *>(Qt), q_off, static_cast<const uint16_t *>(D), d_off, d_clamp0, entries, items,
                       istart + n_d, (int)E, n_q, m, n_d, out_scores, (long long)ld_scores, flags, status);
    hipLaunchKernelGGL(msim::cand_poison_kernel, dim3(eblocks), dim3(256), 0, st, status, n_q, m, out_scores, (long long)ld_scores);
    e = hipGetLastError();
    if (e != hipSuccess) return fail(MSIM_ELAUNCH, "%s: scoring kernel launch: %s", who, hipGetErrorString(e));
    return MSIM_OK;
}

}

extern "C" {

size_t msim_fwd_candidates_workspace_bytes(int n_q, int m, int n_d) {
    if (n_q <= 0 || m <= 0 || n_d < 0) return 0;
    return cand_layout(n_q, m, n_d).total;
}

int msim_fwd_candidates(int dtype, const void *Qt, const int32_t *q_off, const int32_t *q_off_host, int n_q, const void *D,
                        const int32_t *d_off, const uint8_t *d_clamp0, int n_d, int dim, const int64_t *cand, int m, int64_t ld_cand,
                        int64_t id_base, float *out_scores, int64_t ld_scores, int64_t *out_ids, unsigned flags, void *workspace,
                        void *stream) {
    return fwd_candidates("msim_fwd_candidates", msim::kDim, dtype, Qt, q_off, q_off_host, n_q, D, d_off, d_clamp0, n_d, dim, cand, m,
                          ld_cand, id_base, out_scores, ld_scores, out_ids, flags, workspace, stream);
}

size_t msim_fwd_candidates_wide_workspace_bytes(int n_q, int m, int n_d, int dim) {
    (void)dim;
    if (n_q <= 0 || m <= 0 || n_d < 0) return 0;
    return cand_layout(n_q, m, n_d).total;
}

int msim_fwd_candidates_wide(int dtype, const void *Qt, const int32_t *q_off, const int32_t *q_off_host, int n_q, const void *D,
                             const int32_t *d_off, const uint8_t *d_clamp0, int n_d, int dim, const int64_t *cand, int m,
                             int64_t ld_cand, int64_t id_base, float *out_scores, int64_t ld_scores, int64_t *out_ids, unsigned flags,
                             void *workspace, void *stream) {
    return fwd_candidates("msim_fwd_candidates_wide", kCandWideDim, dtype, Qt, q_off, q_off_host, n_q, D, d_off, d_clamp0, n_d, dim, cand,
                          m, ld_cand, id_base, out_scores, ld_scores, out_ids, flags, workspace, stream);
}

}
```

colpali_amd/csrc/maxsim_stream.hip:

```cpp
#pragma once
#include <type_traits>

#include "maxsim_common.hpp"

namespace msim {

struct StreamArgs {
    long long ld;
    FlatQ fq;
    int n_q;
    int n_d;
    unsigned flags;
};

constexpr unsigned kFlagRefBf16 = 1u;
constexpr unsigned kFlagPartial = 2u;

constexpr int kStreamMaxUnits = 8;
constexpr int kStreamTokBytes = kStreamMaxUnits * kUnitTok * 16 + 64;

template <int N>
__device__ __forceinline__ void wait_vmcnt() {
    asm volatile("s_waitcnt vmcnt(%0)" ::"n"(N) : "memory");
}

template <int NU, int RING, bool F16, int AUX = 0, bool IL = false>
__global__ __launch_bounds__(256, 2) void maxsim_stream_kernel(const uint16_t *__restrict__ Qt,
                                                            const uint16_t *__restrict__ D,
                                                            const int32_t *__restrict__ d_off,
                                                            const uint8_t *__restrict__ clamp0,
                                                            float *__restrict__ scores,
                                                            StreamArgs a) {
    extern __shared__ __attribute__((aligned(16))) char smem[];
    const int lane = threadIdx.x & 63;
    const int wave = __builtin_amdgcn_readfirstlane(threadIdx.x >> 6);
    char *ring = smem + wave * (RING * kSlabBytes);
    char *tokmax = smem + 4 * (RING * kSlabBytes) + wave * kStreamTokBytes;
    const int gw = blockIdx.x * 4 + wave;
    const int GW = gridDim.x * 4;

    const int n_tok = flat_qoff(a.fq, a.n_q);
    QueryUnit qu[NU];
#pragma unroll
    for (int u = 0; u < NU; ++u) load_query_unit(qu[u], Qt, u * kUnitTok, n_tok, lane, true);
    int *const rtab = reinterpret_cast<int *>(tokmax + kStreamMaxUnits * kUnitTok * 16);
    if ((lane >> 3) < a.n_q) {
        rtab[2 * (lane >> 3)] = flat_qoff(a.fq, lane >> 3);
        rtab[2 * (lane >> 3) + 1] = flat_qoff(a.fq, (lane >> 3) + 1);
    }

    wait_vmcnt<0>();
#pragma unroll
    for (int u = 0; u < NU; ++u)
#pragma unroll
        for (int ks = 0; ks < kKSteps16; ++ks) asm volatile("" : "+v"(qu[u].f[ks]));

    const int l16 = lane & 15, l4 = lane >> 4;
    int src_off[4];
#pragma unroll
    for (int j = 0; j < 4; ++j) src_off[j] = l4 * kRowBytes + (((l16 ^ l4) ^ (j << 2)) << 4);
    int rd_off[2][kKSteps16];
    slab_rd_offsets16(lane, rd_off);

    int p_idx = gw, p_row = 0, p_len = 0;
    __amdgpu_buffer_rsrc_t p_rsrc = __builtin_amdgcn_make_buffer_rsrc((void *)D, 0, 0, 0x00020000);
    auto p_open = [&]() {
        while (p_idx < a.n_d) {
            const int r0 = d_off[p_idx], r1 = d_off[p_idx + 1];
            p_len = r1 - r0;
            if (p_len > 0) {
                p_rsrc = __builtin_amdgcn_make_buffer_rsrc((void *)(D + (size_t)r0 * kDim), 0,
                                                           p_len * kRowBytes, 0x00020000);
                p_row = 0;
                return;
            }
            p_idx += GW;
        }
    };
    p_open();
    int p_slot = 0;
    auto produce = [&]() -> bool {
        if (p_idx >= a.n_d) return false;
        char *dst = ring + p_slot * kSlabBytes;
        const int soff = p_row * kRowBytes;
#pragma unroll
        for (int i = 0; i < 8; ++i)
            __builtin_amdgcn_raw_ptr_buffer_load_lds(p_rsrc, MSIM_LDS(dst + i * 1024), 16, src_off[i & 3],
                                                     soff + i * 1024, 0, AUX);
        p_slot = (p_slot + 1 == RING) ? 0 : p_slot + 1;
        p_row += kSlabRows;
        if (p_row >= p_len) {
            p_idx += GW;
            p_open();
        }
        return true;
    };

    const __amdgpu_buffer_rsrc_t null_rsrc = __builtin_amdgcn_make_buffer_rsrc((void *)D, 0, 0, 0x00020000);
    auto advance = [&](bool live) {
        p_slot = (p_slot + 1 == RING) ? 0 : p_slot + 1;
        if (live) {
            p_row += kSlabRows;
            if (p_row >= p_len) {
                p_idx += GW;
                p_open();
            }
        }
    };
    if constexpr (IL) {
#pragma unroll
        for (int k = 0; k < RING - 1; ++k) {
            const bool live = p_idx < a.n_d;
            const __amdgpu_buffer_rsrc_t rs = live ? p_rsrc : null_rsrc;
            char *dst = ring + p_slot * kSlabBytes;
            const int soff = live ? p_row * kRowBytes : 0;
#pragma unroll
            for (int i = 0; i < 8; ++i)
                __builtin_amdgcn_raw_ptr_buffer_load_lds(rs, MSIM_LDS(dst + i * 1024), 16, src_off[i & 3], soff + i * 1024, 0, AUX);
            advance(live);
        }
    } else {
#pragma unroll
        for (int i = 0; i < RING - 1; ++i) produce();
    }

    const bool ref_bf16 = (a.flags & kFlagRefBf16) != 0;
    int c_slot = 0;
    for (int c_idx = gw; c_idx < a.n_d; c_idx += GW) {
        const int len = d_off[c_idx + 1] - d_off[c_idx];
        float m[NU];
#pragma unroll
        for (int u = 0; u < NU; ++u) m[u] = -INFINITY;

        auto slab = [&](auto tail_c, int rows_left) {
            constexpr bool kTail = decltype(tail_c)::value;
            bool nx_live = false;
            char *nx_dst = ring;
            int nx_soff = 0;
            __amdgpu_buffer_rsrc_t nx_rsrc = p_rsrc;
            if constexpr (IL) {
                wait_vmcnt<8 * (RING - 2)>();
                nx_live = p_idx < a.n_d;
                nx_dst = ring + p_slot * kSlabBytes;
                nx_soff = nx_live ? p_row * kRowBytes : 0;
                nx_rsrc = nx_live ? p_rsrc : null_rsrc;
            } else {
                const bool issued = produce();
                if (issued)
                    wait_vmcnt<8 * (RING - 1)>();
                else
                    wait_vmcnt<0>();
            }

            const char *src = ring + c_slot * kSlabBytes;
            c_slot = (c_slot + 1 == RING) ? 0 : c_slot + 1;
            bf16x8 af[2][kKSteps16];
#pragma unroll
            for (int g = 0; g < 2; ++g)
#pragma unroll
                for (int ks = 0; ks < kKSteps16; ++ks) af[g][ks] = *reinterpret_cast<const bf16x8 *>(src + rd_off[g][ks]);
            slab_units<F16, NU, kTail, true>(m, af, qu, rows_left, lane, [&](int mf) {
                if constexpr (IL) {
                    if (mf % NU == 0) {
                        const int i = mf / NU;
                        __builtin_amdgcn_raw_ptr_buffer_load_lds(nx_rsrc, MSIM_LDS(nx_dst + i * 1024), 16, src_off[i & 3],
                                                                 nx_soff + i * 1024, 0, AUX);
                    }
                }
            });
            if constexpr (IL) advance(nx_live);
        };
        const int n_full = len / kSlabRows, rem = len - n_full * kSlabRows;
        for (int s = 0; s < n_full; ++s) slab(std::false_type{}, kSlabRows);
        if (rem > 0) slab(std::true_type{}, rem);

        bool clamp = false;
        if (clamp0 != nullptr) {
            const uint64_t addr = reinterpret_cast<uint64_t>(clamp0) + (uint64_t)c_idx;
            clamp = ((scalar_load_u32(addr & ~3ull) >> ((addr & 3) * 8)) & 0xffu) != 0;
        }
#pragma unroll
        for (int u = 0; u < NU; ++u) store_token_max(tokmax, u, m[u], lane);
        int ln = lane;
        asm volatile("" : "+v"(ln));
        const int rq = ln >> 3, ri = ln & 7;
        if (rq < a.n_q) {
            float tot = reduce_query_tokens<F16>(tokmax, rtab[2 * rq], rtab[2 * rq + 1], ri, clamp, ref_bf16);
            if (ref_bf16 && !(a.flags & kFlagPartial)) tot = round_to_input<F16>(tot);
            if (ri == 0) scores[(size_t)rq * a.ld + c_idx] = tot;
        }
    }
}

}
```

colpali_amd/scoring.py:

```python
from __future__ import annotations

import logging
import os
from typing import List, Optional, Union

import torch

from . import _lib
from .corpus import (PackedCorpus, PackedQueries, _check_embeddings, _staging, _widen, block_clamp0, check_query_list, copy_stream,
                     host_list_image, pack_passages, pack_queries)

logger = logging.getLogger(__name__)


def get_torch_device(device: str = "auto") -> str:
    if device == "auto":
        if torch.cuda.is_available():
            device = "cuda:0"
        elif torch.backends.mps.is_available():
            device = "mps"
        else:
            device = "cpu"
        logger.info(f"Using device: {device}")
    return device


def _require_gpu(device: Union[str, torch.device]) -> torch.device:
    dev = torch.device(device)
    if dev.type != "cuda":
        raise RuntimeError(
            f"colpali_amd: this entry point runs on an AMD Instinct MI355X only (requested device: {dev}); "
            "score_multi_vector and score_single_vector have a host path (device='cpu'; it lives in the same library, which links "
            "the HIP runtime: the ROCm user-space libraries must be installed even on a GPU-less host), nothing else does.")
    if not torch.cuda.is_available():
        raise RuntimeError("colpali_amd: no ROCm GPU is visible to torch")
    return dev


def _host_threads() -> int:
    return max(1, min(int(os.environ.get("COLPALI_AMD_HOST_THREADS", "0")) or min(torch.get_num_threads(), _lib.effective_cpus()), 256))


def _score_on_host(qs, ps, batch_size: int, ref_rounding: bool) -> torch.Tensor:
    import numpy as np

    from .corpus import block_clamp0

    L = _lib.lib()

    def rows_of(x, what):
        if isinstance(x, torch.Tensor):
            if x.dim() != 3:
                raise ValueError(f"a {what} tensor must be 3-D (n, max_len, dim)")
            _check_embeddings(x, what)
            t = x.to("cpu").contiguous()
            n, ln, dim = t.shape
            step = ln * dim * t.element_size()
            return [t], np.asarray([t.data_ptr() + i * step for i in range(n)], dtype=np.uint64), np.full(n, ln, dtype=np.int64), dim, t.dtype
        keep = []
        for t in x:
            if t.dim() != 2:
                raise ValueError(f"each {what[:-1] if what.endswith('s') else what} must be 2-D (sequence_length, dim)")
            _check_embeddings(t, what)
            if t.dtype != x[0].dtype:
                raise RuntimeError(f"expected {what} of one dtype, got {x[0].dtype} and {t.dtype}")
            if t.shape[1] != x[0].shape[1]:
                raise RuntimeError(f"expected {what} of one embedding width, got {x[0].shape[1]} and {t.shape[1]}")
            keep.append(t.to("cpu").contiguous())
        return (keep, np.asarray([t.data_ptr() if t.numel() else 0 for t in keep], dtype=np.uint64),
                np.asarray([t.shape[0] for t in keep], dtype=np.int64), int(x[0].shape[1]), x[0].dtype)

    q_keep, q_ptr, q_rows, q_dim, q_dtype = rows_of(qs, "queries")
    p_keep, p_ptr, p_rows, p_dim, p_dtype = rows_of(ps, "passages")
    if q_dtype != p_dtype:
        raise RuntimeError(f"expected queries and passages of one dtype, got {q_dtype} and {p_dtype}")
    if q_dim != p_dim:
        raise RuntimeError(f"queries have embedding width {q_dim}, the corpus {p_dim}")
    clamp0 = None
    if not isinstance(ps, torch.Tensor):
        lengths = torch.from_numpy(p_rows)
        flags = block_clamp0(lengths, batch_size)
        if bool((lengths == 0).any()):
            for j in range(0, len(p_rows), batch_size):
                if int(lengths[j: j + batch_size].max()) == 0:
                    raise RuntimeError("max(): Expected reduction dim 3 to have non-zero size.")
        clamp0 = flags.numpy() if bool(flags.any()) else None
    n_q, n_d = len(q_rows), len(p_rows)
    out = torch.empty((n_q, n_d), dtype=torch.float32)
    rc = L.msim_fwd_host_lists(_lib.dtype_code(q_dtype), q_ptr.ctypes.data, q_rows.ctypes.data, n_q, p_ptr.ctypes.data,
                               p_rows.ctypes.data, clamp0.ctypes.data if clamp0 is not None else None, n_d, q_dim, out.data_ptr(),
                               out.stride(0) if n_q > 1 else max(n_d, 1), _lib.MSIM_FLAG_REF_ROUNDING if ref_rounding else 0,
                               _host_threads())
    del q_keep, p_keep
    if rc != 0:
        msg = L.msim_host_last_error().decode("utf-8", "replace")
        raise (NotImplementedError if rc == -2 else ValueError if rc == -1 else RuntimeError)(f"msim_fwd_host_lists: {msg}")
    return out


_MAX_FWD_SCRATCH = 1 << 30


def _ref_rounding_from_env() -> bool:
    return os.environ.get("COLPALI_AMD_REF_ROUNDING", "0") not in ("", "0")


def maxsim_scores(queries: Union[torch.Tensor, PackedQueries], corpus: PackedCorpus, *, ref_rounding: bool = False,
                  out: Optional[torch.Tensor] = None, ref_bf16: Optional[bool] = None) -> torch.Tensor:
    if ref_bf16 is not None:
        ref_rounding = ref_bf16
    L = _lib.lib()
    flat = isinstance(queries, PackedQueries)
    if not flat and (queries.dim() != 3 or not queries.is_contiguous()):
        raise ValueError("queries must be a PackedQueries or a contiguous [n_q, Lq, width] tensor")
    if queries.dtype != corpus.blob.dtype:
        raise RuntimeError(f"expected queries and passages of one dtype, got {queries.dtype} and {corpus.blob.dtype}")
    dt = _lib.dtype_code(queries.dtype)
    if queries.device != corpus.device:
        raise ValueError("queries and corpus live on different devices")
    n_q = len(queries)
    dim = queries.tokens.shape[1] if flat else queries.shape[2]
    if dim != corpus.blob.shape[1]:
        raise RuntimeError(f"queries have embedding width {dim}, the corpus {corpus.blob.shape[1]}")
    n = len(corpus)
    if out is None:
        out = torch.empty((n_q, n), dtype=torch.float32, device=queries.device)
    elif out.shape != (n_q, n) or out.dtype != torch.float32 or out.stride(1) != 1:
        raise ValueError("out must be fp32 [n_q, n] with unit inner stride")
    flags = _lib.MSIM_FLAG_REF_ROUNDING if ref_rounding else 0
    if n:
        flags |= min(65535, max(1, corpus.average_rows())) << 8
    ld = out.stride(0) if n_q > 1 else max(n, 1)
    if flat:
        with torch.cuda.device(queries.device):
            oh = queries.offsets_host
            ws = _lib.workspace(L.msim_fwd_ragged_workspace_bytes(dt, oh.data_ptr(), n_q, n, dim), queries.device)
            rc = L.msim_fwd_ragged(dt, _lib.ptr(queries.tokens), _lib.ptr(queries.offsets), oh.data_ptr(), n_q, _lib.ptr(corpus.blob),
                                   _lib.ptr(corpus.offsets), _lib.ptr(corpus.clamp0), n, dim, _lib.ptr(out), ld, flags, _lib.ptr(ws),
                                   _lib.current_stream_handle(queries.device))
            _lib.check(rc, "msim_fwd_ragged")
        return out
    Lq = queries.shape[1]
    ws_bytes = L.msim_fwd_workspace_bytes(dt, n_q, Lq, n, dim)
    group = n_q if ws_bytes <= _MAX_FWD_SCRATCH else max(1, int(n_q * _MAX_FWD_SCRATCH // ws_bytes))
    with torch.cuda.device(queries.device):
        for q0 in range(0, n_q, group):
            nq = min(group, n_q - q0)
            ws = _lib.workspace(L.msim_fwd_workspace_bytes(dt, nq, Lq, n, dim), queries.device)
            rc = L.msim_fwd(dt, _lib.ptr(queries[q0:q0 + nq]), nq, Lq, _lib.ptr(corpus.blob), _lib.ptr(corpus.offsets),
                            _lib.ptr(corpus.clamp0), n, dim, _lib.ptr(out[q0:q0 + nq]), ld,
                            flags, _lib.ptr(ws), _lib.current_stream_handle(queries.device))
            _lib.check(rc, "msim_fwd")
    return out


def score_multi_vector(
    qs: Union[torch.Tensor, List[torch.Tensor]],
    ps: Union[torch.Tensor, List[torch.Tensor]],
    batch_size: int = 128,
    device: Optional[Union[str, torch.device]] = None,
) -> torch.Tensor:
    device = device or get_torch_device("auto")
    if len(qs) == 0:
        raise ValueError("No queries provided")
    if len(ps) == 0:
        raise ValueError("No passages provided")
    ref_rounding = _ref_rounding_from_env()
    if torch.device(device).type == "cpu":
        scores = _score_on_host(qs, ps, batch_size, ref_rounding)
        assert scores.shape[0] == len(qs), f"Expected {len(qs)} scores, got {scores.shape[0]}"
        return scores
    dev = _require_gpu(device)
    with _lib.on_gpu_local_cpus(dev):
        checked = False
        if not isinstance(ps, torch.Tensor):
            if not isinstance(qs, torch.Tensor):
                check_query_list(qs)
                checked = True
            elif qs.dim() != 3:
                raise ValueError("a query tensor must be 3-D (n_queries, max_len, dim)")
            scores = _score_host_list_pipelined(qs, ps, dev, batch_size, ref_rounding, checked)
            if scores is not None:
                assert scores.shape[0] == len(qs), f"Expected {len(qs)} scores, got {scores.shape[0]}"
                return scores
        q = pack_queries(qs, dev, _checked=checked)
        cols = []
        for lo, hi in passage_ranges(ps, batch_size, _corpus_budget_bytes(dev)):
            corpus = pack_passages(ps[lo:hi], dev, batch_size=batch_size)
            cols.append(maxsim_scores(q, corpus, ref_rounding=ref_rounding).cpu())
            del corpus
    scores = cols[0] if len(cols) == 1 else torch.cat(cols, dim=1)
    assert scores.shape[0] == len(qs), f"Expected {len(qs)} scores, got {scores.shape[0]}"
    return scores.to(torch.float32)


TIMELINE = None


def _stamp(label: str) -> None:
    if TIMELINE is not None:
        import time

        TIMELINE.append((label, time.perf_counter()))


_PIPE_RANGE_BYTES = 48 << 20


def _score_host_list_pipelined(qs, ps, dev: torch.device, batch_size: int, ref_rounding: bool, qs_checked: bool = False) -> Optional[torch.Tensor]:
    import numpy as np

    _stamp("begin")
    info = host_list_image(ps)
    if info is None:
        return None
    keep, srcs, rows, dim, dtype = info
    q_is_box = isinstance(qs, torch.Tensor)
    q_dtype = qs.dtype if q_is_box else qs[0].dtype
    q_dim = int(qs.shape[2]) if q_is_box else int(qs[0].shape[1])
    if q_is_box:
        _check_embeddings(qs, "queries")
    if q_dtype != dtype:
        raise RuntimeError(f"expected queries and passages of one dtype, got {q_dtype} and {dtype}")
    if _lib.kernel_width(dim, dtype) != dim:
        return None
    n = len(keep)
    row_bytes = dim * keep[0].element_size()
    prefix = np.zeros(n + 1, dtype=np.int64)
    np.cumsum(rows * row_bytes, out=prefix[1:])
    total = int(prefix[n])
    total_rows = total // row_bytes
    if total == 0 or total > _corpus_budget_bytes(dev) or total_rows >= 2**31:
        return None
    lengths = torch.from_numpy(rows)
    flags = block_clamp0(lengths, batch_size)
    if bool((rows == 0).any()):
        for j in range(0, n, batch_size):
            if int(rows[j: j + batch_size].max()) == 0:
                raise RuntimeError("max(): Expected reduction dim 3 to have non-zero size.")
    n_q = len(qs)
    if q_dim != dim:
        raise RuntimeError(f"queries have embedding width {q_dim}, the corpus {dim}")
    _lib.place_gather_threads(dev, srcs[:: max(1, n // 8)][:8])
    _stamp("checked")
    main = torch.cuda.current_stream(dev)
    side = copy_stream(dev)
    n_blocks = (n + batch_size - 1) // batch_size
    n_sub = max(1, min(n_blocks, 8, total // _PIPE_RANGE_BYTES))
    cuts = sorted({min(n, ((n_blocks * i + n_sub - 1) // n_sub) * batch_size) for i in range(1, n_sub + 1)} | {n})
    state = [0, 0]
    dv = {}

    with torch.cuda.device(dev):

        def prepare() -> torch.Tensor:
            dv["q"] = pack_queries(qs, dev, _checked=qs_checked)
            blob = torch.empty((total_rows, dim), dtype=dtype, device=dev)
            blob.record_stream(side)
            off_host = torch.zeros(n + 1, dtype=torch.int32)
            off_host[1:] = torch.from_numpy((prefix[1:] // row_bytes).astype(np.int32))
            dv["blob"] = blob
            dv["offsets"] = off_host.to(dev, non_blocking=True)
            dv["clamp0"] = flags.to(dev, non_blocking=True) if bool(flags.any()) else None
            dv["out"] = torch.empty((n_q, n), dtype=torch.float32, device=dev)
            side.wait_stream(main)
            _stamp("prepared")
            return blob.view(torch.uint8).view(-1)

        def score_arrived(bytes_done: int) -> None:
            q, blob, offsets, clamp0, out = dv["q"], dv["blob"], dv["offsets"], dv["clamp0"], dv["out"]
            while state[1] < len(cuts) and int(prefix[cuts[state[1]]]) <= bytes_done:
                lo, hi = state[0], cuts[state[1]]
                ev = torch.cuda.Event()
                ev.record(side)
                main.wait_event(ev)
                if hi > lo:
                    part = PackedCorpus(blob=blob, offsets=offsets[lo:hi + 1], clamp0=None if clamp0 is None else clamp0[lo:hi],
                                        lengths=lengths[lo:hi], avg_rows=max(1, int(rows[lo:hi].sum()) // (hi - lo)))
                    maxsim_scores(q, part, ref_rounding=ref_rounding, out=out[:, lo:hi])
                state[0] = hi
                state[1] += 1

        _staging.of(dev).upload_image(srcs, prefix, n, None, side, on_chunk=score_arrived, prepare=prepare)
        _stamp("issued")
        scores = dv["out"].cpu()
        _stamp("done")
    del keep
    return scores


def _corpus_budget_bytes(dev: torch.device) -> int:
    mb = os.environ.get("COLPALI_AMD_CORPUS_BUDGET_MB")
    if mb:
        return int(mb) << 20
    free, _ = torch.cuda.mem_get_info(dev)
    return int(free * 0.6)


def passage_ranges(ps, batch_size: int, budget_bytes: int):
    n = len(ps)
    if isinstance(ps, torch.Tensor):
        per = [ps.shape[1] * ps.shape[2] * ps.element_size()] * n
    else:
        per = [p.shape[0] * p.shape[1] * p.element_size() for p in ps]
    if sum(per) <= budget_bytes:
        return [(0, n)]
    ranges, lo, acc = [], 0, 0
    for b0 in range(0, n, batch_size):
        blk = sum(per[b0 : b0 + batch_size])
        if acc and acc + blk > budget_bytes:
            ranges.append((lo, b0))
            lo, acc = b0, 0
        acc += blk
    ranges.append((lo, n))
    return ranges


def similarity_matrix(a: torch.Tensor, b: torch.Tensor, *, ref_rounding: bool = False,
                      out: Optional[torch.Tensor] = None) -> torch.Tensor:
    L = _lib.lib()
    if a.dim() != 2 or b.dim() != 2 or a.shape[1] != b.shape[1]:
        raise ValueError("expected [n_a, dim] and [n_b, dim]")
    if a.dtype != b.dtype:
        raise RuntimeError(f"expected both operands of one dtype, got {a.dtype} and {b.dtype}")
    if a.device.type != "cuda" or b.device != a.device:
        raise RuntimeError("colpali_amd.similarity_matrix runs on an MI355X only (no CPU fallback)")
    _check_embeddings(a, "similarity operand")
    aw, bw = _widen(a).contiguous(), _widen(b).contiguous()
    n_a, n_b = a.shape[0], b.shape[0]
    if out is None:
        out = torch.empty((n_a, n_b), dtype=torch.float32, device=a.device)
    elif out.shape != (n_a, n_b) or out.dtype != torch.float32 or (n_b > 1 and out.stride(1) != 1):
        raise ValueError("out must be fp32 [n_a, n_b] with unit inner stride")
    with torch.cuda.device(a.device):
        rc = L.msim_sim_matrix(_lib.dtype_code(a.dtype), _lib.ptr(aw), n_a, _lib.ptr(bw), n_b, aw.shape[1], _lib.ptr(out),
                               out.stride(0) if n_a > 1 else max(n_b, 1),
                               _lib.MSIM_FLAG_REF_ROUNDING if ref_rounding else 0, _lib.current_stream_handle(a.device))
    _lib.check(rc, "msim_sim_matrix")
    return out


def score_single_vector(
    qs: Union[torch.Tensor, List[torch.Tensor]],
    ps: Union[torch.Tensor, List[torch.Tensor]],
    device: Optional[Union[str, torch.device]] = None,
) -> torch.Tensor:
    device = device or get_torch_device("auto")
    if isinstance(qs, list) and isinstance(ps, list):
        if len(qs) == 0:
            raise ValueError("No queries provided")
        if len(ps) == 0:
            raise ValueError("No passages provided")
        qs, ps = torch.stack(qs), torch.stack(ps)
    if torch.device(device).type == "cpu":
        a, b = qs.to("cpu"), ps.to("cpu")
        if a.dim() != 2 or b.dim() != 2 or a.shape[1] != b.shape[1]:
            raise ValueError("expected [n_a, dim] and [n_b, dim]")
        if a.dtype != b.dtype:
            raise RuntimeError(f"expected both operands of one dtype, got {a.dtype} and {b.dtype}")
        _check_embeddings(a, "similarity operand")
        a, b = a.contiguous(), b.contiguous()
        L = _lib.lib()
        scores = torch.empty((a.shape[0], b.shape[0]), dtype=torch.float32)
        rc = L.msim_sim_matrix_host(_lib.dtype_code(a.dtype), a.data_ptr(), a.shape[0], b.data_ptr(), b.shape[0], a.shape[1],
                                    scores.data_ptr(), max(b.shape[0], 1), 0, _host_threads())
        if rc != 0:
            raise RuntimeError(f"msim_sim_matrix_host: {L.msim_host_last_error().decode('utf-8', 'replace')}")
        assert scores.shape[0] == len(qs), f"Expected {len(qs)} scores, got {scores.shape[0]}"
        return scores
    dev = _require_gpu(device)
    scores = similarity_matrix(qs.to(dev), ps.to(dev))
    assert scores.shape[0] == len(qs), f"Expected {len(qs)} scores, got {scores.shape[0]}"
    return scores.to(torch.float32)


def get_similarity_maps_from_embeddings(image_embeddings: torch.Tensor, query_embeddings: torch.Tensor, n_patches,
                                        image_mask: torch.Tensor) -> List[torch.Tensor]:
    if isinstance(n_patches, tuple):
        n_patches = [n_patches] * image_embeddings.size(0)
    maps: List[torch.Tensor] = []
    for idx in range(image_embeddings.size(0)):
        nx, ny = n_patches[idx]
        if image_mask[idx].sum() != nx * ny:
            raise ValueError(
                f"The number of patches ({nx} x {ny} = {nx * ny}) "
                f"does not match the number of non-padded image tokens ({image_mask[idx].sum()}).")
        patches = image_embeddings[idx][image_mask[idx]]
        sim = similarity_matrix(query_embeddings[idx].contiguous(), patches.contiguous())
        maps.append(sim.view(-1, ny, nx).permute(0, 2, 1).to(image_embeddings.dtype))
    return maps
```

include/maxsim.h:

```cpp
#ifndef COLPALI_AMD_MAXSIM_H
#define COLPALI_AMD_MAXSIM_H

#include <stddef.h>
#include <stdint.h>

#ifdef __cplusplus
extern "C" {
#endif

#define MSIM_ABI_VERSION 22

#define MSIM_OK 0
#define MSIM_EINVAL (-1)
#define MSIM_EUNSUPPORTED (-2)
#define MSIM_ELAUNCH (-3)

#define MSIM_DTYPE_BF16 0
#define MSIM_DTYPE_F16 1
#define MSIM_DTYPE_F32 2

#define MSIM_FLAG_REF_ROUNDING 0x1u

#define MSIM_FLAG_AVG_ROWS(n) ((uint32_t)((n) < 0 ? 0 : ((n) > 65535 ? 65535 : (n))) << 8)

int msim_abi_version(void);
const char *msim_last_error(void);

size_t msim_fwd_workspace_bytes(int dtype, int n_q, int Lq, int n_d, int dim);

int msim_fwd(int dtype, const void *Q, int n_q, int Lq,
                  const void *D, const int32_t *d_off, const uint8_t *d_clamp0,
                  int n_d, int dim,
                  float *scores, int64_t ld_scores,
                  uint32_t flags, void *workspace, void *stream);

const char *msim_host_last_error(void);
int msim_fwd_host(int dtype, const void *Q, int n_q, int Lq,
                  const void *D, const int32_t *d_off, const uint8_t *d_clamp0,
                  int n_d, int dim,
                  float *scores, int64_t ld_scores,
                  uint32_t flags, int n_threads);
int msim_fwd_host_lists(int dtype, const void *const *q_ptr, const int64_t *q_rows, int n_q,
                        const void *const *d_ptr, const int64_t *d_rows, const uint8_t *d_clamp0,
                        int n_d, int dim,
                        float *scores, int64_t ld_scores,
                        uint32_t flags, int n_threads);
int msim_sim_matrix_host(int dtype, const void *A, int n_a, const void *B, int n_b, int dim,
                         float *out, int64_t ld_out, uint32_t flags, int n_threads);

int msim_fwd_plan(const int32_t *q_off_host, int n_q, int Lq, int32_t *out5);
size_t msim_fwd_ragged_workspace_bytes(int dtype, const int32_t *q_off_host, int n_q, int n_d, int dim);
int msim_fwd_ragged(int dtype, const void *Qt, const int32_t *q_off, const int32_t *q_off_host, int n_q,
                    const void *D, const int32_t *d_off, const uint8_t *d_clamp0,
                    int n_d, int dim,
                    float *scores, int64_t ld_scores,
                    uint32_t flags, void *workspace, void *stream);

size_t msim_fwd_candidates_workspace_bytes(int n_q, int m, int n_d);
int msim_fwd_candidates(int dtype, const void *Qt, const int32_t *q_off, const int32_t *q_off_host, int n_q,
                        const void *D, const int32_t *d_off, const uint8_t *d_clamp0, int n_d, int dim,
                        const int64_t *cand, int m, int64_t ld_cand, int64_t id_base,
                        float *out_scores, int64_t ld_scores, int64_t *out_ids ,
                        unsigned flags, void *workspace, void *stream);

size_t msim_fwd_candidates_wide_workspace_bytes(int n_q, int m, int n_d, int dim);
int msim_fwd_candidates_wide(int dtype, const void *Qt, const int32_t *q_off, const int32_t *q_off_host, int n_q,
                             const void *D, const int32_t *d_off, const uint8_t *d_clamp0, int n_d, int dim,
                             const int64_t *cand, int m, int64_t ld_cand, int64_t id_base,
                             float *out_scores, int64_t ld_scores, int64_t *out_ids ,
                             unsigned flags, void *workspace, void *stream);

int msim_align_candidates(int dtype, const void *Qt, const int32_t *q_off, int n_q, int64_t q_rows, int max_q_tokens,
                          const void *D, const int32_t *d_off, const uint8_t *d_clamp0, int n_d, int64_t d_rows, int dim,
                          const int64_t *cand, int m, int64_t ld_cand, int64_t id_base,
                          float *best_sim, int32_t *best_row,
                          float *sims , int max_rows,
                          void *stream);

int msim_fwd_transposed(int dtype, const void *Q, int n_q, int Lq, const void *D, int n_d, int Ld, int dim,
                        float *scores, int64_t ld_scores, int32_t *q_lengths, void *stream);

int msim_dense_t_supported(int dtype, int n_q, int Lq, int n_d, int Ld, int dim);
size_t msim_dense_t_route_bytes(int n_q, int Lq, int n_d);
int msim_fwd_transposed_route(int dtype, const void *Q, int n_q, int Lq, const void *D, int n_d, int Ld, int dim,
                              float *scores, int64_t ld_scores, int32_t *q_lengths, uint8_t *route, void *stream);
size_t msim_dense_t_bwd_workspace_bytes(int n_q, int Lq, int n_d, int Ld, int dim);
int msim_dense_t_bwd(int dtype, const void *Q, int n_q, int Lq, const void *D, int n_d, int Ld, int dim,
                     const float *G, int64_t ldg, const void *g_scale, int g_scale_dtype, const uint8_t *route,
                     void *dQ, void *dD, void *workspace, void *stream);

int msim_query_compact(const void *box, int n_q, int Lq, int row_bytes, const int32_t *q_off, int32_t *counts, void *out,
                       void *stream);
int msim_host_count_nonzero_rows(const void *const *src, const int64_t *rows, int64_t row_bytes, int64_t n, int32_t *counts,
                                 int n_threads);
int msim_host_gather_nonzero_rows(void *dst, const void *const *src, const int64_t *rows, int64_t row_bytes,
                                  const int64_t *dst_row, int64_t n, int n_threads);

int msim_pairs_argmax(int dtype, const void *Q, int n_q, int Lq,
                      const void *D, const int32_t *d_off, const uint8_t *d_clamp0,
                      int n_d, int dim, int max_doc_rows,
                      const int32_t *pairs, int n_pairs,
                      float *out_scores, int32_t *out_argmax, void *stream);

int msim_allpairs_argmax(int dtype, const void *Q, int n_q, int Lq,
                         const void *D, const int32_t *d_off, const uint8_t *d_clamp0, int n_d, int dim,
                         float *out_scores, int64_t ld_scores, int32_t *out_argmax, void *stream);

size_t msim_pairs_bwd_workspace_bytes(int n_q, int Lq, int n_d, int dim, int max_doc_rows, int n_pairs);
int msim_pairs_bwd(int dtype, const void *Q, int n_q, int Lq,
                   const void *D, const int32_t *d_off, int n_d, int dim, int max_doc_rows,
                   const int32_t *pairs, const int32_t *order_by_doc,
                   const float *g, const void *g_scale, int g_scale_dtype,
                   const int32_t *argmax, int n_pairs,
                   int out_dtype, void *dQ, void *dD, void *workspace, void *stream);

int msim_smooth_fwd(int dtype, const void *Q, int n_q, int Lq,
                    const void *D, const int32_t *d_off, int n_d, int dim, float tau,
                    float *scores, int64_t ld_scores, void *stream);
int msim_smooth_pairs(int dtype, const void *Q, int n_q, int Lq,
                      const void *D, const int32_t *d_off, int n_d, int dim,
                      const int32_t *pairs, int n_pairs, float tau,
                      float *out_scores, float *out_lse, void *stream);
size_t msim_smooth_bwd_workspace_bytes(int n_q, int Lq, int dim);
int msim_smooth_pairs_bwd(int dtype, const void *Q, int n_q, int Lq,
                          const void *D, const int32_t *d_off, int n_d, int dim, int max_doc_rows,
                          const int32_t *pairs, const int32_t *order_by_doc,
                          const float *g, const float *lse, int n_pairs, float tau,
                          float *dQ, float *dD, void *workspace, void *stream);

#define MSIM_LOSS_PAIRWISE 0
#define MSIM_LOSS_INFONCE 1
#define MSIM_LOSS_SIGMOID 2
size_t msim_loss_epilogue_workspace_bytes(int B, int C);
int msim_loss_epilogue(int mode, const float *scores, int64_t ld, int B, int C,
                       const void *Q, int q_dtype, int Lq, int width, int offset,
                       float temperature, int normalize, int filter, float filter_threshold, float filter_factor,
                       float *G, int32_t *pairs, float *coef, int32_t *order,
                       void *workspace, float *out, void *loss_out, const int32_t *q_lengths, void *stream);

int msim_embed_head(int dtype, const void *X, int64_t M, int H,
                    const void *W, const void *bias, int n_out,
                    const int32_t *row_map, void *out, int64_t ld_out, void *stream);

int msim_embed_head_row_map(const void *mask, int mask_kind, const void *extra, int extra_kind, int64_t M, int32_t *row_map, void *stream);

int msim_embed_head_writer_map(const void *mask, int mask_kind, const void *extra, int extra_kind, int B, int S, const int64_t *rows_before,
                               int64_t *counts, int32_t *row_map, int64_t *rows_after, void *stream);

int msim_embed_head_bwd(int dtype, const void *proj, const void *grad_out, const int32_t *row_map, int64_t M, int n_out,
                        void *dproj, void *stream);

int msim_sim_matrix(int dtype, const void *A, int n_a, const void *B, int n_b, int dim,
                    float *out, int64_t ld_out, uint32_t flags, void *stream);

int msim_pool_cluster(int dtype, const void *E, const int32_t *d_off, int n_pages, int dim, int max_rows,
                      const int64_t *ws_off, int pool_factor, float *X_ws, double *D_ws,
                      int32_t *labels, int32_t *n_clusters, void *stream);
int msim_pool_reduce(int dtype, const void *E, const int32_t *d_off, int n_pages, int dim, int ld_in,
                     const int32_t *labels, const int32_t *out_off, void *out, int ld_out, void *stream);

int msim_host_gather(void *dst, const void *const *src, const int64_t *dst_off, const int64_t *nbytes, int64_t n, int n_threads);
int msim_host_gather_range(void *dst, const void *const *src, const int64_t *prefix, int64_t n, int64_t lo, int64_t hi, int n_threads);
int msim_host_gather_range_begin(void *dst, const void *const *src, const int64_t *prefix, int64_t n, int64_t lo, int64_t hi, int n_threads);
int msim_host_gather_range_wait(void);
int msim_host_threads_affinity(const int32_t *cpus, int n_cpus);

size_t msim_topk_workspace_bytes(int n_q, int64_t n, int k);
int msim_topk_f32(const float *scores, const int64_t *ids, int n_q, int64_t n, int64_t ld,
                  int k, int64_t id_base,
                  float *out_scores, int64_t *out_ids, void *workspace, void *stream);

int msim_fde_encode_docs(int dtype, const void *D, const int32_t *d_off, int n_d, int64_t n_rows, int dim,
                         const float *G, const float *S, int reps, int ksim, int dproj, int fill_empty,
                         void *out, uint8_t *codes , void *stream);
int msim_fde_encode_queries(int dtype, const void *Qt, const int32_t *q_off, int n_q, int64_t n_rows, int dim,
                            const float *G, const float *S, int reps, int ksim, int dproj,
                            void *out, uint8_t *codes , void *stream);
int msim_fde_scores(int dtype, const void *Fq, int n_q, const void *Fd, int n_d, int F, float *scores, int64_t ld_scores,
                    void *stream);

int msim_i8_encode_docs(int dtype, const void *D, const int32_t *d_off, int n_d, int64_t n_rows, int dim,
                        int8_t *codes, float *scales, void *stream);
int msim_i8_encode_queries(int dtype, const void *Qt, int64_t n_rows, int dim, int8_t *codes, float *scales, void *stream);
int msim_i8_scores(const int8_t *q8, const float *sq, const int32_t *q_off, int n_q, int64_t q_rows, int max_q_tokens,
                   const int8_t *d8, const float *sd, const int32_t *d_off, const uint8_t *clamp0 , int n_d,
                   int64_t d_rows, int dim, float *scores, int64_t ld_scores, void *stream);

int msim_cent_encode_docs(int dtype, const void *D, const int32_t *d_off, int n_d, int64_t n_rows, int dim, int max_doc_rows,
                          const void *C, int K, uint16_t *codes, int32_t *status , void *stream);
size_t msim_cent_table_bytes(int n_q, int max_q_tokens, int K);
int msim_cent_table(int dtype, const void *Qt, const int32_t *q_off, int n_q, int64_t q_rows, int max_q_tokens, int dim,
                    const void *C, int K, void *table, void *stream);
int msim_cent_scores_plan(int n_q, int max_q_tokens, int K, int n_d, int64_t d_rows, int32_t *plan );
int msim_cent_scores(const void *table, const int32_t *q_off, int n_q, int64_t q_rows, int max_q_tokens, int K,
                     const uint16_t *codes, const int32_t *d_off, const uint8_t *clamp0 , int n_d, int64_t d_rows,
                     float *scores, int64_t ld_scores, void *stream);

int msim_res_encode_docs(int dtype, const void *D, int64_t n_rows, int dim, const uint16_t *codes, const void *C, int K,
                         const float *cutoffs, int bits, uint8_t *residuals, void *stream);
int msim_res_decode_rows(int dtype, const uint16_t *codes, const uint8_t *residuals, int64_t n_rows, int64_t row0, int64_t row1,
                         const void *C, int K, const float *weights, int bits, int dim, void *out, void *stream);
size_t msim_res_candidates_workspace_bytes(int n_q, int m, int n_d);
int msim_res_candidates(int dtype, const void *Qt, const int32_t *q_off, const int32_t *q_off_host, int n_q, const uint16_t *codes,
                        const uint8_t *residuals, const void *C, int K, const float *weights, int bits, const int32_t *d_off,
                        const uint8_t *d_clamp0 , int n_d, int64_t d_rows, int dim, const int64_t *cand, int m,
                        int64_t ld_cand, int64_t id_base, float *out_scores, int64_t ld_scores, int64_t *out_ids ,
                        void *workspace, void *stream);
size_t msim_res_scores_workspace_bytes(int n_q, int n_d);
int msim_res_scores(int dtype, const void *Qt, const int32_t *q_off, const int32_t *q_off_host, int n_q, const uint16_t *codes,
                    const uint8_t *residuals, const void *C, int K, const float *weights, int bits, const int32_t *d_off,
                    const uint8_t *d_clamp0 , int n_d, int64_t d_rows, int dim, float *out_scores, int64_t ld_scores,
                    void *workspace, void *stream);

size_t msim_live_compact_workspace_bytes(int n_slots, int64_t bounce_bytes);
int msim_live_compact(void *rows, int64_t row_bytes, int64_t rows_bound, int32_t *off, const uint8_t *alive, int n_slots,
                      int64_t *rows_used_out, void *workspace, void *bounce, int64_t bounce_bytes, void *stream);
int msim_live_mask_scores(float *scores, int64_t ld, int n_q, int64_t n, const uint8_t *alive, void *stream);

int msim_mine_bounds(const float *scores, int64_t ld, int n_q, int64_t n, const int64_t *pos_ids, const int32_t *pos_off, int64_t nnz,
                     int64_t id_base, const uint8_t *alive , int local, float *bounds, void *stream);
int msim_mine_mask(float *scores, int64_t ld, int n_q, int64_t n, const float *bounds , float max_ratio,
                   const uint8_t *alive , const int64_t *pos_ids, const int32_t *pos_off, int64_t nnz, int64_t id_base,
                   void *stream);
int msim_gather_pages(const void *rows, int64_t row_bytes, int64_t d_rows, const int32_t *d_off, int n_d, int64_t id_base,
                      const int64_t *ids, int64_t n_slots, int64_t pad_rows, void *out, int32_t *lengths, void *stream);

int msim_filter_pack(const uint8_t *mask, int64_t ld_mask, int rows, int64_t n, uint32_t *words, int64_t ld_words, void *stream);
int msim_filter_mask(float *scores, int64_t ld, int n_q, int64_t n, const uint32_t *bits , int64_t ld_words,
                     const int32_t *page_labels , const int32_t *query_labels ,
                     const uint8_t *alive , void *stream);
size_t msim_filter_list_workspace_bytes(int n_q, int64_t n);
int msim_filter_list(const uint32_t *bits , int64_t ld_words, const int32_t *page_labels ,
                     const int32_t *query_labels , const uint8_t *alive , int n_q, int64_t n,
                     int64_t id_base, int64_t *cand, int64_t ld_cand, int m_cap, int32_t *counts, void *workspace, void *stream);
int msim_filter_ids(int64_t *ids, int64_t ld, int n_q, int64_t m, int64_t n, int64_t id_base, const uint32_t *bits ,
                    int64_t ld_words, const int32_t *page_labels , const int32_t *query_labels ,
                    const uint8_t *alive , void *stream);

#define MSIM_GROUP_THREAD_MAX 16
#define MSIM_GROUP_WAVE_MAX 1024
#define MSIM_GROUP_SELECT_MAX_M 4096
#define MSIM_GROUP_SELECT_MAX_K 1024
int msim_group_reduce(const float *scores, int64_t ld, int n_q, int64_t n, const int32_t *offsets, const int32_t *pages, int n_groups,
                      int64_t id_base, float *group_scores, int64_t *group_pages, int64_t ld_out, void *stream);
int msim_group_select(const float *scores, const int64_t *gids, const int64_t *pages, int n_q, int m, int64_t ld, int k,
                      float *out_scores, int64_t *out_gids, int64_t *out_pages, void *stream);

#ifdef __cplusplus
}
#endif
#endif
```

Before: 103.5 million pairs/s.

## Stream corpus from a lossless 13-bit packed image with flagged-doc fallback

Adds an encoder that repacks the resident bf16 corpus into 13-bit slabs: 8 low mantissa bits, a 4-bit nibble and a sign bit, with fixed exponent high bits implied. Documents holding values that cannot be represented this way are flagged. A new streaming kernel reads the smaller image, and a list-driven pass of the original kernel rescores the flagged documents. The aim is to cut HBM bytes per scan in this bandwidth-bound MaxSim. The cost is extra device memory for the image, a one-off encode after the corpus is seen twice, and decode arithmetic inside the kernel.

```diff
diff --git a/colpali_amd/_lib.py b/colpali_amd/_lib.py
--- a/colpali_amd/_lib.py
+++ b/colpali_amd/_lib.py
@@ -82,6 +82,16 @@
     L.msim_fwd_ragged_workspace_bytes.restype = sz
     L.msim_fwd_ragged.argtypes = [i32, vp, vp, vp, i32, vp, vp, vp, i32, i32, vp, i64, u32, vp, vp]
     L.msim_fwd_ragged.restype = i32
+    L.msim_pack13_image_bytes.argtypes = [i64]
+    L.msim_pack13_image_bytes.restype = sz
+    L.msim_pack13_encode.argtypes = [vp, vp, vp, i32, i64, vp, vp, vp, vp, vp]
+    L.msim_pack13_encode.restype = i32
+    L.msim_pack13_decode.argtypes = [vp, vp, vp, i32, i64, vp, vp]
+    L.msim_pack13_decode.restype = i32
+    L.msim_fwd_pack13.argtypes = [i32, vp, i32, i32, vp, vp, vp, i32, i32, vp, vp, vp, vp, i32, vp, i64, u32, vp, vp]
+    L.msim_fwd_pack13.restype = i32
+    L.msim_fwd_ragged_pack13.argtypes = [i32, vp, vp, vp, i32, vp, vp, vp, i32, i32, vp, vp, vp, vp, i32, vp, i64, u32, vp, vp]
+    L.msim_fwd_ragged_pack13.restype = i32
     L.msim_query_compact.argtypes = [vp, i32, i32, i32, vp, vp, vp, vp]
     L.msim_query_compact.restype = i32
     L.msim_host_count_nonzero_rows.argtypes = [vp, vp, i64, i64, vp, i32]
diff --git a/colpali_amd/corpus.py b/colpali_amd/corpus.py
--- a/colpali_amd/corpus.py
+++ b/colpali_amd/corpus.py
@@ -4,7 +4,7 @@
 import operator
 import os
 import threading
-from dataclasses import dataclass
+from dataclasses import dataclass, field
 from typing import List, Optional, Sequence, Union
 
 import numpy as np
@@ -35,6 +35,27 @@
     return torch.from_numpy(flags.astype(np.uint8))
 
 
+PACK13_SLAB_BYTES = 6656
+PACK13_MAX_FLAGGED = 0.05
+PACK13_RESERVE_BYTES = 2 << 30
+
+
+def _pack13_env() -> Optional[bool]:
+    v = os.environ.get("COLPALI_AMD_PACK13", "")
+    return None if v == "" else v != "0"
+
+
+@dataclass
+class Pack13Image:
+    key: tuple
+    image: torch.Tensor
+    slab_off: torch.Tensor
+    flagged: torch.Tensor
+    ids: Optional[torch.Tensor]
+    n_flagged: int
+    n_slabs: int
+
+
 @dataclass
 class PackedCorpus:
     blob: torch.Tensor
@@ -43,9 +64,58 @@
     lengths: torch.Tensor
     id_base: int = 0
     avg_rows: Optional[int] = None
+    _pack13: Optional[Pack13Image] = field(default=None, compare=False, repr=False)
+    _pack13_note: Optional[tuple] = field(default=None, compare=False, repr=False)
 
     def __len__(self) -> int:
         return int(self.lengths.numel())
+
+    def _pack13_key(self) -> tuple:
+        b, o = self.blob, self.offsets
+        return (b.data_ptr(), b._version, o.data_ptr(), o._version, tuple(b.shape), tuple(o.shape))
+
+    def _pack13_eligible(self) -> bool:
+        return (self.blob.dtype == torch.bfloat16 and self.blob.dim() == 2 and self.blob.shape[1] == EMBED_DIM
+                and self.blob.device.type == "cuda" and len(self) > 0)
+
+    def pack13(self) -> bool:
+        key = self._pack13_key()
+        if self._pack13 is not None and self._pack13.key == key:
+            return True
+        self._pack13 = None
+        if _pack13_env() is False or not self._pack13_eligible():
+            return False
+        self._pack13 = _pack13_build(self, key)
+        self._pack13_note = None if self._pack13 is not None else (key, "declined")
+        return self._pack13 is not None
+
+    def drop_pack13(self) -> None:
+        self._pack13 = None
+        self._pack13_note = None
+
+    def _pack13_for_scan(self) -> Optional[Pack13Image]:
+        env = _pack13_env()
+        if env is False:
+            self._pack13 = None
+            return None
+        key = self._pack13_key()
+        img = self._pack13
+        if img is not None:
+            if img.key == key:
+                return img
+            self._pack13 = None
+            self._pack13_note = None
+        if not self._pack13_eligible() or torch.cuda.is_current_stream_capturing():
+            return None
+        note = self._pack13_note
+        if note is not None and note[0] == key:
+            if note[1] == "declined":
+                return None
+        elif not env:
+            self._pack13_note = (key, "seen")
+            return None
+        self.pack13()
+        return self._pack13
 
     def average_rows(self) -> int:
         if self.avg_rows is None:
@@ -73,6 +143,54 @@
     @property
     def nbytes(self) -> int:
         return self.blob.numel() * self.blob.element_size()
+
+
+def _pack13_build(corpus: "PackedCorpus", key: tuple) -> Optional[Pack13Image]:
+    L = _lib_mod.lib()
+    n = len(corpus)
+    dev = corpus.blob.device
+    ln = corpus.lengths.detach().to("cpu").numpy().astype(np.int64, copy=False)
+    slab_off = np.zeros(n + 1, dtype=np.int64)
+    np.cumsum((ln + 31) // 32, out=slab_off[1:])
+    n_slabs = int(slab_off[-1])
+    if n_slabs == 0 or n_slabs >= 2**31:
+        return None
+    with torch.cuda.device(dev):
+        if not np.array_equal(np.diff(corpus.offsets.detach().to("cpu").numpy().astype(np.int64)), ln):
+            return None
+        need = int(L.msim_pack13_image_bytes(n_slabs))
+        free, _total = torch.cuda.mem_get_info(dev)
+        free += torch.cuda.memory_reserved(dev) - torch.cuda.memory_allocated(dev)
+        if free - need < PACK13_RESERVE_BYTES:
+            return None
+        try:
+            image = torch.empty((need,), dtype=torch.uint8, device=dev)
+        except RuntimeError:
+            return None
+        slab_off_d = torch.from_numpy(slab_off.astype(np.int32)).to(dev)
+        flagged = torch.empty((n,), dtype=torch.uint8, device=dev)
+        ids = torch.empty((n,), dtype=torch.int32, device=dev)
+        count = torch.empty((1,), dtype=torch.int32, device=dev)
+        _lib_mod.check(L.msim_pack13_encode(_lib_mod.ptr(corpus.blob), _lib_mod.ptr(corpus.offsets), _lib_mod.ptr(slab_off_d), n, n_slabs,
+                                            _lib_mod.ptr(image), _lib_mod.ptr(flagged), _lib_mod.ptr(ids), _lib_mod.ptr(count),
+                                            _lib_mod.current_stream_handle(dev)), "msim_pack13_encode")
+        n_flagged = int(count.item())
+    if n_flagged > PACK13_MAX_FLAGGED * n:
+        return None
+    return Pack13Image(key=key, image=image, slab_off=slab_off_d, flagged=flagged,
+                       ids=ids[:n_flagged].clone() if n_flagged else None, n_flagged=n_flagged, n_slabs=n_slabs)
+
+
+def pack13_decode(corpus: "PackedCorpus") -> torch.Tensor:
+    img = corpus._pack13
+    if img is None:
+        raise ValueError("the corpus holds no 13-bit image")
+    out = torch.zeros_like(corpus.blob)
+    with torch.cuda.device(corpus.blob.device):
+        _lib_mod.check(_lib_mod.lib().msim_pack13_decode(_lib_mod.ptr(img.image), _lib_mod.ptr(corpus.offsets), _lib_mod.ptr(img.slab_off),
+                                                         len(corpus), img.n_slabs, _lib_mod.ptr(out),
+                                                         _lib_mod.current_stream_handle(corpus.blob.device)), "msim_pack13_decode")
+    return out
 
 
 def _check_embeddings(x: torch.Tensor, what: str) -> None:
diff --git a/colpali_amd/csrc/abi_pack13.hip b/colpali_amd/csrc/abi_pack13.hip
--- /dev/null
+++ b/colpali_amd/csrc/abi_pack13.hip
@@ -0,0 +1,43 @@
+#include <hip/hip_runtime.h>
+
+#include "../../include/maxsim.h"
+#include "abi_common.hpp"
+#include "pack13.hip"
+
+using namespace msim_abi;
+
+extern "C" {
+
+size_t msim_pack13_image_bytes(int64_t n_slabs) { return n_slabs <= 0 ? 0 : (size_t)n_slabs * msim::kSlab13Bytes; }
+
+int msim_pack13_encode(const void *D, const int32_t *d_off, const int32_t *slab_off, int n_d, int64_t n_slabs, void *image,
+                       uint8_t *flags, int32_t *list, int32_t *count, void *stream) {
+    if (n_d < 0 || n_slabs < 0 || n_slabs > 0x7fffffff) return fail(MSIM_EINVAL, "msim_pack13_encode: bad size (n_d=%d n_slabs=%lld)", n_d, (long long)n_slabs);
+    if (!count || (n_d > 0 && (!d_off || !slab_off || !flags || !list)) || (n_slabs > 0 && (!D || !image)))
+        return fail(MSIM_EINVAL, "msim_pack13_encode: null pointer argument");
+    if (misaligned(D, 16) || misaligned(image, 16)) return fail(MSIM_EINVAL, "msim_pack13_encode: D and image must be 16-byte aligned");
+    hipStream_t st = static_cast<hipStream_t>(stream);
+    if (hipMemsetAsync(count, 0, sizeof(int32_t), st) != hipSuccess || (n_d > 0 && hipMemsetAsync(flags, 0, (size_t)n_d, st) != hipSuccess))
+        return fail(MSIM_ELAUNCH, "msim_pack13_encode: hipMemsetAsync failed");
+    if (n_d == 0) return MSIM_OK;
+    if (n_slabs > 0) {
+        hipLaunchKernelGGL(msim::pack13_encode_kernel, dim3((unsigned)n_slabs), dim3(128), 0, st, static_cast<const uint16_t *>(D), d_off,
+                           slab_off, n_d, static_cast<uint8_t *>(image), flags);
+        if (int rc = launch_failed("pack13_encode_kernel")) return rc;
+    }
+    hipLaunchKernelGGL(msim::pack13_list_kernel, dim3(1), dim3(1024), 0, st, flags, n_d, list, count);
+    return launch_failed("pack13_list_kernel");
+}
+
+int msim_pack13_decode(const void *image, const int32_t *d_off, const int32_t *slab_off, int n_d, int64_t n_slabs, void *out,
+                       void *stream) {
+    if (n_d < 0 || n_slabs < 0 || n_slabs > 0x7fffffff) return fail(MSIM_EINVAL, "msim_pack13_decode: bad size (n_d=%d n_slabs=%lld)", n_d, (long long)n_slabs);
+    if (n_d == 0 || n_slabs == 0) return MSIM_OK;
+    if (!image || !d_off || !slab_off || !out) return fail(MSIM_EINVAL, "msim_pack13_decode: null pointer argument");
+    if (misaligned(out, 16) || misaligned(image, 16)) return fail(MSIM_EINVAL, "msim_pack13_decode: out and image must be 16-byte aligned");
+    hipLaunchKernelGGL(msim::pack13_decode_kernel, dim3((unsigned)n_slabs), dim3(128), 0, static_cast<hipStream_t>(stream),
+                       static_cast<const uint8_t *>(image), d_off, slab_off, n_d, static_cast<uint16_t *>(out));
+    return launch_failed("pack13_decode_kernel");
+}
+
+}
diff --git a/colpali_amd/csrc/maxsim_abi.hip b/colpali_amd/csrc/maxsim_abi.hip
--- a/colpali_amd/csrc/maxsim_abi.hip
+++ b/colpali_amd/csrc/maxsim_abi.hip
@@ -10,6 +10,7 @@
 #include "abi_common.hpp"
 #include "abi_shapes.hpp"
 #include "maxsim_stream.hip"
+#include "maxsim_stream13.hip"
 #include "maxsim_batch.hip"
 #if defined(MSIM_AB) || defined(MSIM_TRACE)
 #include "maxsim_batch_packed.hip"
@@ -23,6 +24,14 @@
 using namespace msim_abi;
 
 namespace {
+
+struct Pack13View {
+    const uint8_t *image;
+    const int32_t *slab_off;
+    const uint8_t *flagged;
+    const int32_t *list;
+    int n_list;
+};
 
 struct FwdCall {
     const uint16_t *Q, *D;
@@ -39,6 +48,7 @@
     const int32_t *q_off_host = nullptr;
     int seg = 0, n_seg = 1;
     int avg_rows = 0;
+    const Pack13View *p13 = nullptr;
 };
 
 constexpr size_t kFwdWorkspaceBytes = 4096;
@@ -64,9 +74,9 @@
     return v;
 }
 
-template <int NU, bool F16, int AUX, bool IL, int RING = kStreamRing>
-int launch_stream_aux(const FwdCall &c) {
-    auto kern = msim::maxsim_stream_kernel<NU, RING, F16, AUX, IL>;
+template <int NU, bool F16, int AUX, bool IL, int RING = kStreamRing, bool LIST = false>
+int launch_stream_aux(const FwdCall &c, const int32_t *doc_list = nullptr) {
+    auto kern = msim::maxsim_stream_kernel<NU, RING, F16, AUX, IL, LIST>;
     constexpr int lds = 4 * (RING * msim::kSlabBytes + msim::kStreamTokBytes);
     static std::atomic<int> configured[kMaxDevices];
     if (int rc = allow_lds(kern, lds, configured)) return rc;
@@ -79,7 +89,7 @@
     const int wg_needed = (c.n_d + 3) / 4;
     const int wg_cap = c.di->cus * (c.di->lds_per_cu / lds);
     hipLaunchKernelGGL(kern, dim3(wg_needed < wg_cap ? wg_needed : wg_cap), dim3(256), lds, c.st, c.Q, c.D, c.d_off,
-                       c.clamp0, c.scores, a);
+                       c.clamp0, c.scores, a, doc_list);
     hipError_t e = hipGetLastError();
     if (e != hipSuccess) return fail(MSIM_ELAUNCH, "maxsim_stream_kernel<%d> launch: %s", NU, hipGetErrorString(e));
     return MSIM_OK;
@@ -103,6 +113,33 @@
     }
 #endif
     return launch_stream_aux<NU, F16, 2, true, ring_default>(c);
+}
+
+template <int NU>
+int launch_stream13(const FwdCall &c) {
+    constexpr int RING = NU >= 5 ? 2 : kStreamRing;
+    auto kern = msim::maxsim_stream13_kernel<NU, RING, 2>;
+    constexpr int lds = 4 * (RING * msim::kSlab13Bytes + msim::kStreamTokBytes);
+    static std::atomic<int> configured[kMaxDevices];
+    if (int rc = allow_lds(kern, lds, configured)) return rc;
+    msim::StreamArgs a;
+    a.ld = c.ld;
+    a.fq = flat_q(c);
+    a.n_q = c.n_q;
+    a.n_d = c.n_d;
+    a.flags = c.flags;
+    const int wg_needed = (c.n_d + 3) / 4;
+    const int wg_cap = c.di->cus * (c.di->lds_per_cu / lds);
+    hipLaunchKernelGGL(kern, dim3(wg_needed < wg_cap ? wg_needed : wg_cap), dim3(256), lds, c.st, c.Q, c.d_off, c.clamp0, c.scores, a,
+                       c.p13->image, c.p13->slab_off, c.p13->flagged);
+    hipError_t e = hipGetLastError();
+    if (e != hipSuccess) return fail(MSIM_ELAUNCH, "maxsim_stream13_kernel<%d> launch: %s", NU, hipGetErrorString(e));
+    if (c.p13->n_list > 0) {
+        FwdCall l = c;
+        l.n_d = c.p13->n_list;
+        return launch_stream_aux<NU, false, 2, true, RING, true>(l, c.p13->list);
+    }
+    return MSIM_OK;
 }
 
 struct FlatPlan {
@@ -329,6 +366,20 @@
     thread_local FlatPlan plan;
     if (int rc = flat_plan(host_q(c), c.n_q, plan)) return rc;
     if (plan.stream) {
+        if constexpr (!F16) {
+            if (c.p13 != nullptr) {
+                switch (plan.nu) {
+                    case 1: return launch_stream13<1>(c);
+                    case 2: return launch_stream13<2>(c);
+                    case 3: return launch_stream13<3>(c);
+                    case 4: return launch_stream13<4>(c);
+                    case 5: return launch_stream13<5>(c);
+                    case 6: return launch_stream13<6>(c);
+                    case 7: return launch_stream13<7>(c);
+                    default: return launch_stream13<8>(c);
+                }
+            }
+        }
         switch (plan.nu) {
             case 1: return launch_stream<1, F16>(c);
             case 2: return launch_stream<2, F16>(c);
@@ -601,9 +652,51 @@
     return tpq > 2 || (Lq % msim::kTokTile) != 0;
 }
 
+int fwd_ragged_impl(int dtype, const void *Qt, const int32_t *q_off, const int32_t *q_off_host, int n_q, const void *D,
+                    const int32_t *d_off, const uint8_t *d_clamp0, int n_d, int dim, float *scores, int64_t ld_scores,
+                    uint32_t flags, void *workspace, void *stream, const Pack13View *p13);
+int fwd_impl(int dtype, const void *Q, int n_q, int Lq, const void *D, const int32_t *d_off, const uint8_t *d_clamp0,
+             int n_d, int dim, float *scores, int64_t ld_scores, uint32_t flags, void *workspace, void *stream, const Pack13View *p13);
+
+int check_pack13(const char *who, const void *image, const int32_t *slab_off, const uint8_t *flagged, const int32_t *list, int n_list,
+                 Pack13View *v) {
+    if (!image || !slab_off || !flagged || n_list < 0 || (n_list > 0 && !list)) return fail(MSIM_EINVAL, "%s: bad image arguments", who);
+    if (reinterpret_cast<uintptr_t>(image) & 15) return fail(MSIM_EINVAL, "%s: the image must be 16-byte aligned", who);
+    *v = Pack13View{static_cast<const uint8_t *>(image), slab_off, flagged, list, n_list};
+    return MSIM_OK;
+}
+
 }
 
 extern "C" {
+
+int msim_fwd_pack13(int dtype, const void *Q, int n_q, int Lq, const void *D, const int32_t *d_off, const uint8_t *d_clamp0, int n_d,
+                    int dim, const void *image, const int32_t *slab_off, const uint8_t *flagged, const int32_t *list, int n_list,
+                    float *scores, int64_t ld_scores, uint32_t flags, void *workspace, void *stream) {
+    Pack13View v;
+    if (int rc = check_pack13("msim_fwd_pack13", image, slab_off, flagged, list, n_list, &v)) return rc;
+    return fwd_impl(dtype, Q, n_q, Lq, D, d_off, d_clamp0, n_d, dim, scores, ld_scores, flags, workspace, stream, &v);
+}
+
+int msim_fwd_ragged_pack13(int dtype, const void *Qt, const int32_t *q_off, const int32_t *q_off_host, int n_q, const void *D,
+                           const int32_t *d_off, const uint8_t *d_clamp0, int n_d, int dim, const void *image, const int32_t *slab_off,
+                           const uint8_t *flagged, const int32_t *list, int n_list, float *scores, int64_t ld_scores, uint32_t flags,
+                           void *workspace, void *stream) {
+    Pack13View v;
+    if (int rc = check_pack13("msim_fwd_ragged_pack13", image, slab_off, flagged, list, n_list, &v)) return rc;
+    return fwd_ragged_impl(dtype, Qt, q_off, q_off_host, n_q, D, d_off, d_clamp0, n_d, dim, scores, ld_scores, flags, workspace, stream, &v);
+}
+
+int msim_fwd_ragged(int dtype, const void *Qt, const int32_t *q_off, const int32_t *q_off_host, int n_q, const void *D,
+                    const int32_t *d_off, const uint8_t *d_clamp0, int n_d, int dim, float *scores, int64_t ld_scores,
+                    uint32_t flags, void *workspace, void *stream) {
+    return fwd_ragged_impl(dtype, Qt, q_off, q_off_host, n_q, D, d_off, d_clamp0, n_d, dim, scores, ld_scores, flags, workspace, stream, nullptr);
+}
+
+int msim_fwd(int dtype, const void *Q, int n_q, int Lq, const void *D, const int32_t *d_off, const uint8_t *d_clamp0,
+             int n_d, int dim, float *scores, int64_t ld_scores, uint32_t flags, void *workspace, void *stream) {
+    return fwd_impl(dtype, Q, n_q, Lq, D, d_off, d_clamp0, n_d, dim, scores, ld_scores, flags, workspace, stream, nullptr);
+}
 
 size_t msim_fwd_workspace_bytes(int dtype, int n_q, int Lq, int n_d, int dim) {
     if (n_q <= 0 || n_d <= 0 || Lq <= 0) return 0;
@@ -636,9 +729,13 @@
     return flat_workspace_bytes(HostQ{q_off_host, 0, 0, 1}, n_q);
 }
 
-int msim_fwd_ragged(int dtype, const void *Qt, const int32_t *q_off, const int32_t *q_off_host, int n_q, const void *D,
+}
+
+namespace {
+
+int fwd_ragged_impl(int dtype, const void *Qt, const int32_t *q_off, const int32_t *q_off_host, int n_q, const void *D,
                     const int32_t *d_off, const uint8_t *d_clamp0, int n_d, int dim, float *scores, int64_t ld_scores,
-                    uint32_t flags, void *workspace, void *stream) {
+                    uint32_t flags, void *workspace, void *stream, const Pack13View *p13) {
     if (n_q < 0 || n_d < 0) return fail(MSIM_EINVAL, "negative size (n_q=%d n_d=%d)", n_q, n_d);
     if (n_q == 0 || n_d == 0) return MSIM_OK;
     if (!scores || !Qt || !D || !d_off || !q_off || !q_off_host) return fail(MSIM_EINVAL, "null pointer argument");
@@ -684,11 +781,12 @@
         }
         return dtype == MSIM_DTYPE_F16 ? launch_batch_panels_flat<true>(c) : launch_batch_panels_flat<false>(c);
     }
+    c.p13 = p13;
     return dtype == MSIM_DTYPE_F16 ? fwd_dispatch<true>(c) : fwd_dispatch<false>(c);
 }
 
-int msim_fwd(int dtype, const void *Q, int n_q, int Lq, const void *D, const int32_t *d_off, const uint8_t *d_clamp0,
-             int n_d, int dim, float *scores, int64_t ld_scores, uint32_t flags, void *workspace, void *stream) {
+int fwd_impl(int dtype, const void *Q, int n_q, int Lq, const void *D, const int32_t *d_off, const uint8_t *d_clamp0,
+             int n_d, int dim, float *scores, int64_t ld_scores, uint32_t flags, void *workspace, void *stream, const Pack13View *p13) {
     if (n_q < 0 || n_d < 0 || Lq <= 0) return fail(MSIM_EINVAL, "negative size (n_q=%d n_d=%d Lq=%d)", n_q, n_d, Lq);
     if (n_q == 0 || n_d == 0) return MSIM_OK;
     if (!scores) return fail(MSIM_EINVAL, "null pointer argument");
@@ -792,8 +890,13 @@
     c.avg_rows = avg_rows;
     c.st = static_cast<hipStream_t>(stream);
     c.workspace = workspace;
+    c.p13 = p13;
     return dtype == MSIM_DTYPE_F16 ? fwd_dispatch<true>(c) : fwd_dispatch<false>(c);
 }
+
+}
+
+extern "C" {
 
 int msim_sim_matrix(int dtype, const void *A, int n_a, const void *B, int n_b, int dim, float *out, int64_t ld_out,
                     uint32_t flags, void *stream) {
diff --git a/colpali_amd/csrc/maxsim_stream.hip b/colpali_amd/csrc/maxsim_stream.hip
--- a/colpali_amd/csrc/maxsim_stream.hip
+++ b/colpali_amd/csrc/maxsim_stream.hip
@@ -24,13 +24,14 @@
     asm volatile("s_waitcnt vmcnt(%0)" ::"n"(N) : "memory");
 }
 
-template <int NU, int RING, bool F16, int AUX = 0, bool IL = false>
+template <int NU, int RING, bool F16, int AUX = 0, bool IL = false, bool LIST = false>
 __global__ __launch_bounds__(256, 2) void maxsim_stream_kernel(const uint16_t *__restrict__ Qt,
                                                             const uint16_t *__restrict__ D,
                                                             const int32_t *__restrict__ d_off,
                                                             const uint8_t *__restrict__ clamp0,
                                                             float *__restrict__ scores,
-                                                            StreamArgs a) {
+                                                            StreamArgs a,
+                                                            const int32_t *__restrict__ doc_list = nullptr) {
     extern __shared__ __attribute__((aligned(16))) char smem[];
     const int lane = threadIdx.x & 63;
     const int wave = __builtin_amdgcn_readfirstlane(threadIdx.x >> 6);
@@ -38,6 +39,10 @@
     char *tokmax = smem + 4 * (RING * kSlabBytes) + wave * kStreamTokBytes;
     const int gw = blockIdx.x * 4 + wave;
     const int GW = gridDim.x * 4;
+    auto doc_id = [&](int i) -> int {
+        if constexpr (LIST) return doc_list[i];
+        else return i;
+    };
 
     const int n_tok = flat_qoff(a.fq, a.n_q);
     QueryUnit qu[NU];
@@ -66,7 +71,8 @@
     __amdgpu_buffer_rsrc_t p_rsrc = __builtin_amdgcn_make_buffer_rsrc((void *)D, 0, 0, 0x00020000);
     auto p_open = [&]() {
         while (p_idx < a.n_d) {
-            const int r0 = d_off[p_idx], r1 = d_off[p_idx + 1];
+            const int p_doc = doc_id(p_idx);
+            const int r0 = d_off[p_doc], r1 = d_off[p_doc + 1];
             p_len = r1 - r0;
             if (p_len > 0) {
                 p_rsrc = __builtin_amdgcn_make_buffer_rsrc((void *)(D + (size_t)r0 * kDim), 0,
@@ -126,7 +132,8 @@
 
     const bool ref_bf16 = (a.flags & kFlagRefBf16) != 0;
     int c_slot = 0;
-    for (int c_idx = gw; c_idx < a.n_d; c_idx += GW) {
+    for (int c_pos = gw; c_pos < a.n_d; c_pos += GW) {
+        const int c_idx = doc_id(c_pos);
         const int len = d_off[c_idx + 1] - d_off[c_idx];
         float m[NU];
 #pragma unroll
diff --git a/colpali_amd/csrc/maxsim_stream13.hip b/colpali_amd/csrc/maxsim_stream13.hip
--- /dev/null
+++ b/colpali_amd/csrc/maxsim_stream13.hip
@@ -0,0 +1,172 @@
+#pragma once
+#include "maxsim_stream.hip"
+#include "pack13_format.hpp"
+
+namespace msim {
+
+__device__ __forceinline__ void pack13_interleave(uint32_t H, uint32_t L, int &o0, int &o1) {
+    o0 = (int)__builtin_amdgcn_perm(H, L, 0x05010400u);
+    o1 = (int)__builtin_amdgcn_perm(H, L, 0x07030602u);
+}
+
+__device__ __forceinline__ void pack13_decode_group(bf16x8 (&af)[kKSteps16], const i32x4 &lo01, const i32x4 &lo23, const i32x4 &nib,
+                                                    uint32_t sign) {
+#pragma unroll
+    for (int ks = 0; ks < kKSteps16; ++ks) {
+        i32x4 o;
+#pragma unroll
+        for (int h = 0; h < 2; ++h) {
+            const int q = 2 * ks + h;
+            const uint32_t L = (uint32_t)(ks < 2 ? lo01[2 * ks + h] : lo23[2 * (ks - 2) + h]);
+            uint32_t H = (((uint32_t)nib[ks] >> (4 * h)) & 0x0f0f0f0fu) | 0x30303030u;
+            H |= (sign << q) & 0x80808080u;
+            int o0, o1;
+            pack13_interleave(H, L, o0, o1);
+            o[2 * h] = o0;
+            o[2 * h + 1] = o1;
+        }
+        af[ks] = __builtin_bit_cast(bf16x8, o);
+    }
+}
+
+template <int NU, int RING, int AUX = 2>
+__global__ __launch_bounds__(256, 2) void maxsim_stream13_kernel(const uint16_t *__restrict__ Qt,
+                                                                 const int32_t *__restrict__ d_off,
+                                                                 const uint8_t *__restrict__ clamp0,
+                                                                 float *__restrict__ scores,
+                                                                 StreamArgs a,
+                                                                 const uint8_t *__restrict__ image,
+                                                                 const int32_t *__restrict__ slab_off,
+                                                                 const uint8_t *__restrict__ flagged) {
+    extern __shared__ __attribute__((aligned(16))) char smem[];
+    const int lane = threadIdx.x & 63;
+    const int wave = __builtin_amdgcn_readfirstlane(threadIdx.x >> 6);
+    char *ring = smem + wave * (RING * kSlab13Bytes);
+    char *tokmax = smem + 4 * (RING * kSlab13Bytes) + wave * kStreamTokBytes;
+    const int gw = blockIdx.x * 4 + wave;
+    const int GW = gridDim.x * 4;
+    auto byte_at = [&](const uint8_t *p, int i) -> bool {
+        const uint64_t addr = reinterpret_cast<uint64_t>(p) + (uint64_t)i;
+        return ((scalar_load_u32(addr & ~3ull) >> ((addr & 3) * 8)) & 0xffu) != 0;
+    };
+
+    const int n_tok = flat_qoff(a.fq, a.n_q);
+    QueryUnit qu[NU];
+#pragma unroll
+    for (int u = 0; u < NU; ++u) load_query_unit(qu[u], Qt, u * kUnitTok, n_tok, lane, true);
+    int *const rtab = reinterpret_cast<int *>(tokmax + kStreamMaxUnits * kUnitTok * 16);
+    if ((lane >> 3) < a.n_q) {
+        rtab[2 * (lane >> 3)] = flat_qoff(a.fq, lane >> 3);
+        rtab[2 * (lane >> 3) + 1] = flat_qoff(a.fq, (lane >> 3) + 1);
+    }
+    wait_vmcnt<0>();
+#pragma unroll
+    for (int u = 0; u < NU; ++u)
+#pragma unroll
+        for (int ks = 0; ks < kKSteps16; ++ks) asm volatile("" : "+v"(qu[u].f[ks]));
+
+    const int off16 = lane * 16, off4 = lane * 4;
+
+    int p_idx = gw, p_s = 0, p_n = 0;
+    const __amdgpu_buffer_rsrc_t null_rsrc = __builtin_amdgcn_make_buffer_rsrc((void *)image, 0, 0, 0x00020000);
+    __amdgpu_buffer_rsrc_t p_rsrc = null_rsrc;
+    auto p_open = [&]() {
+        while (p_idx < a.n_d) {
+            const uint64_t fa = reinterpret_cast<uint64_t>(flagged) + (uint64_t)p_idx;
+            uint32_t s0u, s1u, fw;
+            asm volatile("s_load_dword %0, %3, 0x0\n\ts_load_dword %1, %3, 0x4\n\ts_load_dword %2, %4, 0x0\n\ts_waitcnt lgkmcnt(0)"
+                         : "=&s"(s0u), "=&s"(s1u), "=&s"(fw)
+                         : "s"(reinterpret_cast<uint64_t>(slab_off + p_idx)), "s"(fa & ~3ull)
+                         : "memory");
+            const int s0 = (int)s0u, s1 = (int)s1u;
+            p_n = s1 - s0;
+            if (p_n > 0 && ((fw >> ((fa & 3) * 8)) & 0xffu) == 0) {
+                p_rsrc = __builtin_amdgcn_make_buffer_rsrc((void *)(image + (size_t)s0 * kSlab13Bytes), 0, p_n * kSlab13Bytes, 0x00020000);
+                p_s = 0;
+                return;
+            }
+            p_idx += GW;
+        }
+    };
+    p_open();
+    int p_slot = 0;
+    auto advance = [&](bool live) {
+        p_slot = (p_slot + 1 == RING) ? 0 : p_slot + 1;
+        if (live) {
+            if (++p_s >= p_n) {
+                p_idx += GW;
+                p_open();
+            }
+        }
+    };
+    auto piece = [&](const __amdgpu_buffer_rsrc_t &rs, char *dst, int soff, int i) {
+        if (i < 6)
+            __builtin_amdgcn_raw_ptr_buffer_load_lds(rs, MSIM_LDS(dst + i * 1024), 16, off16, soff + i * 1024, 0, AUX);
+        else
+            __builtin_amdgcn_raw_ptr_buffer_load_lds(rs, MSIM_LDS(dst + kSlab13Sign + (i - 6) * 256), 4, off4,
+                                                     soff + kSlab13Sign + (i - 6) * 256, 0, AUX);
+    };
+#pragma unroll
+    for (int k = 0; k < RING - 1; ++k) {
+        const bool live = p_idx < a.n_d;
+        const __amdgpu_buffer_rsrc_t rs = live ? p_rsrc : null_rsrc;
+        char *dst = ring + p_slot * kSlab13Bytes;
+        const int soff = live ? p_s * kSlab13Bytes : 0;
+#pragma unroll
+        for (int i = 0; i < 8; ++i) piece(rs, dst, soff, i);
+        advance(live);
+    }
+
+    const bool ref_bf16 = (a.flags & kFlagRefBf16) != 0;
+    int c_slot = 0;
+    for (int c_idx = gw; c_idx < a.n_d; c_idx += GW) {
+        if (byte_at(flagged, c_idx)) continue;
+        const int len = d_off[c_idx + 1] - d_off[c_idx];
+        float m[NU];
+#pragma unroll
+        for (int u = 0; u < NU; ++u) m[u] = -INFINITY;
+
+        auto slab = [&](auto tail_c, int rows_left) {
+            constexpr bool kTail = decltype(tail_c)::value;
+            wait_vmcnt<8 * (RING - 2)>();
+            const bool nx_live = p_idx < a.n_d;
+            char *nx_dst = ring + p_slot * kSlab13Bytes;
+            const int nx_soff = nx_live ? p_s * kSlab13Bytes : 0;
+            const __amdgpu_buffer_rsrc_t nx_rsrc = nx_live ? p_rsrc : null_rsrc;
+
+            const char *src = ring + c_slot * kSlab13Bytes;
+            c_slot = (c_slot + 1 == RING) ? 0 : c_slot + 1;
+            bf16x8 af[2][kKSteps16];
+#pragma unroll
+            for (int g = 0; g < 2; ++g) {
+                const i32x4 lo01 = *reinterpret_cast<const i32x4 *>(src + (2 * g) * 1024 + off16);
+                const i32x4 lo23 = *reinterpret_cast<const i32x4 *>(src + (2 * g + 1) * 1024 + off16);
+                const i32x4 nib = *reinterpret_cast<const i32x4 *>(src + kSlab13Nib + g * 1024 + off16);
+                const uint32_t sign = *reinterpret_cast<const uint32_t *>(src + kSlab13Sign + g * 256 + off4);
+                pack13_decode_group(af[g], lo01, lo23, nib, sign);
+            }
+            slab_units<false, NU, kTail, true>(m, af, qu, rows_left, lane, [&](int mf) {
+                if (mf % NU == 0) piece(nx_rsrc, nx_dst, nx_soff, mf / NU);
+            });
+            advance(nx_live);
+        };
+        const int n_full = len / kSlabRows, rem = len - n_full * kSlabRows;
+        for (int s = 0; s < n_full; ++s) slab(std::false_type{}, kSlabRows);
+        if (rem > 0) slab(std::true_type{}, rem);
+
+        bool clamp = false;
+        if (clamp0 != nullptr) clamp = byte_at(clamp0, c_idx);
+#pragma unroll
+        for (int u = 0; u < NU; ++u) store_token_max(tokmax, u, m[u], lane);
+        int ln = lane;
+        asm volatile("" : "+v"(ln));
+        const int rq = ln >> 3, ri = ln & 7;
+        if (rq < a.n_q) {
+            float tot = reduce_query_tokens<false>(tokmax, rtab[2 * rq], rtab[2 * rq + 1], ri, clamp, ref_bf16);
+            if (ref_bf16 && !(a.flags & kFlagPartial)) tot = round_to_input<false>(tot);
+            if (ri == 0) scores[(size_t)rq * a.ld + c_idx] = tot;
+        }
+    }
+}
+
+}
diff --git a/colpali_amd/csrc/pack13.hip b/colpali_amd/csrc/pack13.hip
--- /dev/null
+++ b/colpali_amd/csrc/pack13.hip
@@ -0,0 +1,113 @@
+#pragma once
+#include "maxsim_common.hpp"
+#include "pack13_format.hpp"
+
+namespace msim {
+
+
+__device__ __forceinline__ bool pack13_representable(uint32_t u) {
+    const uint32_t e = (u >> 7) & 0xffu;
+    return e >= 96u && e <= 127u;
+}
+
+__device__ __forceinline__ int pack13_doc_of_slab(const int32_t *__restrict__ slab_off, int n_d, int s) {
+    int lo = 0, hi = n_d - 1;
+    while (lo < hi) {
+        const int mid = (lo + hi) >> 1;
+        if (slab_off[mid + 1] > s) hi = mid;
+        else lo = mid + 1;
+    }
+    return lo;
+}
+
+__global__ __launch_bounds__(128) void pack13_encode_kernel(const uint16_t *__restrict__ D, const int32_t *__restrict__ d_off,
+                                                            const int32_t *__restrict__ slab_off, int n_d,
+                                                            uint8_t *__restrict__ image, uint8_t *__restrict__ flags) {
+    const int s = blockIdx.x;
+    const int c = pack13_doc_of_slab(slab_off, n_d, s);
+    const int r0 = d_off[c], len = d_off[c + 1] - r0;
+    const int g = threadIdx.x >> 6, L = threadIdx.x & 63;
+    const int row = (s - slab_off[c]) * kSlabRows + 16 * g + (L & 15);
+    uint32_t low[8], nib[4], sign = 0;
+    bool bad = false;
+#pragma unroll
+    for (int ks = 0; ks < kKSteps16; ++ks) {
+        i32x4 v = i32x4{0, 0, 0, 0};
+        if (row < len) v = *reinterpret_cast<const i32x4 *>(D + (size_t)(r0 + row) * kDim + 32 * ks + 8 * (L >> 4));
+        uint32_t lo0 = 0, lo1 = 0, n = 0;
+#pragma unroll
+        for (int j = 0; j < 8; ++j) {
+            const uint32_t u = ((uint32_t)v[j >> 1] >> (16 * (j & 1))) & 0xffffu;
+            if (row < len && !pack13_representable(u)) bad = true;
+            const uint32_t code_lo = row < len ? (u & 0xffu) : 0u, code_n = row < len ? ((u >> 8) & 0xfu) : 0u;
+            const uint32_t code_s = row < len ? (u >> 15) : 0u;
+            if (j < 4) lo0 |= code_lo << (8 * j);
+            else lo1 |= code_lo << (8 * (j - 4));
+            n |= code_n << (8 * (j & 3) + 4 * (j >> 2));
+            sign |= code_s << (8 * (j & 3) + 7 - (2 * ks + (j >> 2)));
+        }
+        low[2 * ks] = lo0;
+        low[2 * ks + 1] = lo1;
+        nib[ks] = n;
+    }
+    uint8_t *slab = image + (size_t)s * kSlab13Bytes;
+#pragma unroll
+    for (int h = 0; h < 2; ++h)
+        *reinterpret_cast<i32x4 *>(slab + (2 * g + h) * 1024 + 16 * L) =
+            i32x4{(int)low[4 * h], (int)low[4 * h + 1], (int)low[4 * h + 2], (int)low[4 * h + 3]};
+    *reinterpret_cast<i32x4 *>(slab + kSlab13Nib + g * 1024 + 16 * L) = i32x4{(int)nib[0], (int)nib[1], (int)nib[2], (int)nib[3]};
+    *reinterpret_cast<uint32_t *>(slab + kSlab13Sign + g * 256 + 4 * L) = sign;
+    if (bad) flags[c] = 1;
+}
+
+__global__ __launch_bounds__(1024) void pack13_list_kernel(const uint8_t *__restrict__ flags, int n_d, int32_t *__restrict__ list,
+                                                           int32_t *__restrict__ count) {
+    __shared__ int part[1024];
+    const int t = threadIdx.x;
+    const int per = (n_d + 1023) / 1024;
+    const int c0 = t * per < n_d ? t * per : n_d, c1 = c0 + per < n_d ? c0 + per : n_d;
+    int mine = 0;
+    for (int c = c0; c < c1; ++c) mine += flags[c] != 0;
+    part[t] = mine;
+    __syncthreads();
+    for (int d = 1; d < 1024; d <<= 1) {
+        const int v = t >= d ? part[t - d] : 0;
+        __syncthreads();
+        part[t] += v;
+        __syncthreads();
+    }
+    int w = part[t] - mine;
+    for (int c = c0; c < c1; ++c)
+        if (flags[c] != 0) list[w++] = c;
+    if (t == 1023) *count = part[1023];
+}
+
+__global__ __launch_bounds__(128) void pack13_decode_kernel(const uint8_t *__restrict__ image, const int32_t *__restrict__ d_off,
+                                                            const int32_t *__restrict__ slab_off, int n_d, uint16_t *__restrict__ out) {
+    const int s = blockIdx.x;
+    const int c = pack13_doc_of_slab(slab_off, n_d, s);
+    const int r0 = d_off[c], len = d_off[c + 1] - r0;
+    const int g = threadIdx.x >> 6, L = threadIdx.x & 63;
+    const int row = (s - slab_off[c]) * kSlabRows + 16 * g + (L & 15);
+    if (row >= len) return;
+    const uint8_t *slab = image + (size_t)s * kSlab13Bytes;
+    const uint32_t sign = *reinterpret_cast<const uint32_t *>(slab + kSlab13Sign + g * 256 + 4 * L);
+    const i32x4 nib = *reinterpret_cast<const i32x4 *>(slab + kSlab13Nib + g * 1024 + 16 * L);
+#pragma unroll
+    for (int ks = 0; ks < kKSteps16; ++ks) {
+        const i32x4 lw = *reinterpret_cast<const i32x4 *>(slab + (2 * g + (ks >> 1)) * 1024 + 16 * L);
+        uint32_t o[4];
+#pragma unroll
+        for (int j = 0; j < 8; ++j) {
+            const uint32_t lo = ((uint32_t)lw[2 * (ks & 1) + (j >> 2)] >> (8 * (j & 3))) & 0xffu;
+            const uint32_t n = ((uint32_t)nib[ks] >> (8 * (j & 3) + 4 * (j >> 2))) & 0xfu;
+            const uint32_t sg = (sign >> (8 * (j & 3) + 7 - (2 * ks + (j >> 2)))) & 1u;
+            const uint32_t u = (sg << 15) | 0x3000u | (n << 8) | lo;
+            if (j & 1) o[j >> 1] |= u << 16;
+            else o[j >> 1] = u;
+        }
+        *reinterpret_cast<i32x4 *>(out + (size_t)(r0 + row) * kDim + 32 * ks + 8 * (L >> 4)) = i32x4{(int)o[0], (int)o[1], (int)o[2], (int)o[3]};
+    }
+}
+
+}
diff --git a/colpali_amd/csrc/pack13_format.hpp b/colpali_amd/csrc/pack13_format.hpp
--- /dev/null
+++ b/colpali_amd/csrc/pack13_format.hpp
@@ -0,0 +1,8 @@
+#pragma once
+
+namespace msim {
+
+constexpr int kSlab13Bytes = 6656;
+constexpr int kSlab13Nib = 4096, kSlab13Sign = 6144;
+
+}
diff --git a/colpali_amd/scoring.py b/colpali_amd/scoring.py
--- a/colpali_amd/scoring.py
+++ b/colpali_amd/scoring.py
@@ -131,10 +131,23 @@
     if n:
         flags |= min(65535, max(1, corpus.average_rows())) << 8
     ld = out.stride(0) if n_q > 1 else max(n, 1)
+    img = None
+    if n and n_q <= 8 and dim == 128 and queries.dtype == torch.bfloat16 and queries.device.type == "cuda":
+        tokens = int(queries.offsets_host[-1]) if flat else n_q * queries.shape[1]
+        if tokens <= 128:
+            img = corpus._pack13_for_scan()
     if flat:
         with torch.cuda.device(queries.device):
             oh = queries.offsets_host
             ws = _lib.workspace(L.msim_fwd_ragged_workspace_bytes(dt, oh.data_ptr(), n_q, n, dim), queries.device)
+            if img is not None:
+                rc = L.msim_fwd_ragged_pack13(dt, _lib.ptr(queries.tokens), _lib.ptr(queries.offsets), oh.data_ptr(), n_q,
+                                              _lib.ptr(corpus.blob), _lib.ptr(corpus.offsets), _lib.ptr(corpus.clamp0), n, dim,
+                                              _lib.ptr(img.image), _lib.ptr(img.slab_off), _lib.ptr(img.flagged), _lib.ptr(img.ids),
+                                              img.n_flagged, _lib.ptr(out), ld, flags, _lib.ptr(ws),
+                                              _lib.current_stream_handle(queries.device))
+                _lib.check(rc, "msim_fwd_ragged_pack13")
+                return out
             rc = L.msim_fwd_ragged(dt, _lib.ptr(queries.tokens), _lib.ptr(queries.offsets), oh.data_ptr(), n_q, _lib.ptr(corpus.blob),
                                    _lib.ptr(corpus.offsets), _lib.ptr(corpus.clamp0), n, dim, _lib.ptr(out), ld, flags, _lib.ptr(ws),
                                    _lib.current_stream_handle(queries.device))
@@ -147,6 +160,13 @@
         for q0 in range(0, n_q, group):
             nq = min(group, n_q - q0)
             ws = _lib.workspace(L.msim_fwd_workspace_bytes(dt, nq, Lq, n, dim), queries.device)
+            if img is not None:
+                rc = L.msim_fwd_pack13(dt, _lib.ptr(queries[q0:q0 + nq]), nq, Lq, _lib.ptr(corpus.blob), _lib.ptr(corpus.offsets),
+                                       _lib.ptr(corpus.clamp0), n, dim, _lib.ptr(img.image), _lib.ptr(img.slab_off),
+                                       _lib.ptr(img.flagged), _lib.ptr(img.ids), img.n_flagged, _lib.ptr(out[q0:q0 + nq]), ld,
+                                       flags, _lib.ptr(ws), _lib.current_stream_handle(queries.device))
+                _lib.check(rc, "msim_fwd_pack13")
+                continue
             rc = L.msim_fwd(dt, _lib.ptr(queries[q0:q0 + nq]), nq, Lq, _lib.ptr(corpus.blob), _lib.ptr(corpus.offsets),
                             _lib.ptr(corpus.clamp0), n, dim, _lib.ptr(out[q0:q0 + nq]), ld,
                             flags, _lib.ptr(ws), _lib.current_stream_handle(queries.device))
diff --git a/include/maxsim.h b/include/maxsim.h
--- a/include/maxsim.h
+++ b/include/maxsim.h
@@ -55,6 +55,19 @@
                     int n_d, int dim,
                     float *scores, int64_t ld_scores,
                     uint32_t flags, void *workspace, void *stream);
+
+size_t msim_pack13_image_bytes(int64_t n_slabs);
+int msim_pack13_encode(const void *D, const int32_t *d_off, const int32_t *slab_off, int n_d, int64_t n_slabs, void *image,
+                       uint8_t *flagged, int32_t *list, int32_t *count, void *stream);
+int msim_pack13_decode(const void *image, const int32_t *d_off, const int32_t *slab_off, int n_d, int64_t n_slabs, void *out,
+                       void *stream);
+int msim_fwd_pack13(int dtype, const void *Q, int n_q, int Lq, const void *D, const int32_t *d_off, const uint8_t *d_clamp0,
+                    int n_d, int dim, const void *image, const int32_t *slab_off, const uint8_t *flagged, const int32_t *list,
+                    int n_list, float *scores, int64_t ld_scores, uint32_t flags, void *workspace, void *stream);
+int msim_fwd_ragged_pack13(int dtype, const void *Qt, const int32_t *q_off, const int32_t *q_off_host, int n_q, const void *D,
+                           const int32_t *d_off, const uint8_t *d_clamp0, int n_d, int dim, const void *image,
+                           const int32_t *slab_off, const uint8_t *flagged, const int32_t *list, int n_list, float *scores,
+                           int64_t ld_scores, uint32_t flags, void *workspace, void *stream);
 
 size_t msim_fwd_candidates_workspace_bytes(int n_q, int m, int n_d);
 int msim_fwd_candidates(int dtype, const void *Qt, const int32_t *q_off, const int32_t *q_off_host, int n_q,
```

New measurement: 114.3 million pairs/s, median of 6. +10.4%, better.
